# pminervini/hyperopt

Hardware: AMD Instinct MI355X
Metric: EI candidates scored/sec (x components) (higher is better)
Workload: dtype f64 (log-sum-exp: fp64 accumulation, fp32 exp2 of the shifted term, its argument from an fp32 block-local quadratic (mode 3); quantized: fp64 erf); 1 GPU; config 4: 100-D uniform space, 1e4-trial history, 1e7 candidates/suggest (lpdf roofline stress); parallelism=single

## Files before the change

### hyperopt_amd/_engine.py

```python
from __future__ import annotations

import ctypes as C
import os
import threading

import numpy as np

_HERE = os.path.dirname(os.path.abspath(__file__))
LIB_PATH = os.environ.get('TPE_ENGINE_LIB', os.path.join(_HERE, 'libtpe_engine.so'))

TPE_OK = 0
TPE_E_INVALID = -1
TPE_E_BOUNDS = -2
TPE_E_NEGATIVE = -3
TPE_E_NOMEM = -4
TPE_E_HIP = -5
TPE_E_NODEVICE = -6
TPE_E_INDEX = -7

GMM, LGMM, CAT = 0, 1, 2
HAS_LOW, HAS_HIGH, HAS_Q, PCHOICE = 1, 2, 4, 8
OBS_IDENT, OBS_LOG, OBS_LOG_CLIP_EXPLOW, OBS_LOG_CLIP_EPS = 0, 1, 2, 3
KIND_NAMES = ('lse_gmm', 'lse_lgmm', 'erf_gmm', 'erf_lgmm', 'categorical')

EXPORTS = (
    'tpe_version', 'tpe_device_count', 'tpe_create', 'tpe_destroy', 'tpe_last_error',
    'tpe_synchronize', 'tpe_split', 'tpe_parzen_fit', 'tpe_categorical_posterior',
    'tpe_lpdf', 'tpe_score', 'tpe_sample', 'tpe_plan_create', 'tpe_plan_destroy',
    'tpe_plan_num_levels', 'tpe_plan_set_history', 'tpe_plan_fit', 'tpe_plan_get_mixture',
    'tpe_plan_get_table',
    'tpe_plan_suggest', 'tpe_plan_suggest_shard', 'tpe_plan_merge', 'tpe_plan_score_candidates', 'tpe_plan_last_stats',
    'tpe_plan_profile', 'tpe_plan_profile_read', 'tpe_microbench', 'tpe_plan_get_results',
    'tpe_plan_results_device', 'tpe_plan_census', 'tpe_plan_fit_suggest',
    'tpe_plan_set_lattice', 'tpe_plan_update_history', 'tpe_plan_set_prune',
    'tpe_plan_sample_prior', 'tpe_plan_score_candidates_sorted', 'tpe_plan_census_n',
    'tpe_plan_tie_counts', 'tpe_plan_tab_wmax', 'tpe_plan_anneal', 'tpe_plan_anneal_trace',
    'tpe_plan_set_anneal_order', 'tpe_plan_tab_bound', 'tpe_plan_tab_hot',
    'tpe_plan_cand_dump', 'tpe_plan_draw_screen_stats', 'tpe_plan_score_points',
    'tpe_plan_sample_points', 'tpe_plan_topk_points', 'tpe_plan_gather_points',
    'tpe_plan_joint_fit', 'tpe_plan_joint_get_mixture', 'tpe_plan_joint_score_points',
    'tpe_plan_joint_sides', 'tpe_plan_joint_sample_points', 'tpe_math_probe',
    'tpe_plan_group_info', 'tpe_plan_group_fit', 'tpe_plan_group_get_mixture',
    'tpe_plan_group_score_points', 'tpe_plan_group_sides', 'tpe_plan_group_sample_points',
    'tpe_plan_group_batch_points',
    'tpe_plan_set_objectives', 'tpe_plan_pareto_get', 'tpe_plan_pareto_shape',
)

BATCH_MAX = 1024
MAX_OBJ = 8

SHARD_ALIGN = 8192


class EngineUnavailable(RuntimeError):
    """The HIP engine library or an MI355X (gfx950) device is not available."""


class EngineError(RuntimeError):
    pass


class TpeHp(C.Structure):
    _fields_ = [('family', C.c_int32), ('flags', C.c_uint32), ('obs_transform', C.c_int32),
                ('upper', C.c_int32), ('prior_mu', C.c_double), ('prior_sigma', C.c_double),
                ('low', C.c_double), ('high', C.c_double), ('q', C.c_double),
                ('cond_begin', C.c_int32), ('cond_count', C.c_int32),
                ('pprior_begin', C.c_int64)]


class TpeSpace(C.Structure):
    _fields_ = [('n_hp', C.c_int32), ('hp', C.POINTER(TpeHp)), ('n_cond', C.c_int32),
                ('cond_parent', C.POINTER(C.c_int32)), ('cond_branch', C.POINTER(C.c_int32)),
                ('n_pprior', C.c_int64), ('pprior', C.POINTER(C.c_double))]


RESULT_DTYPE = np.dtype([('score', '<f8'), ('value', '<f8'), ('index', '<i8'),
                         ('active', '<i4'), ('pad', '<i4')])
ANNEAL_TRACE_DTYPE = np.dtype([('row', '<i4'), ('rank', '<i4'), ('u', '<f8', (4,))])

_D = C.POINTER(C.c_double)
_lib = None
_lib_lock = threading.Lock()


def _share_hip_runtime():
    if os.environ.get('TPE_ENGINE_HIP_RUNTIME', '') == 'system':
        return
    import importlib.util
    try:
        spec = importlib.util.find_spec('torch')
    except (ImportError, ValueError):
        spec = None
    if spec is None or not spec.origin:
        return
    hip = os.path.join(os.path.dirname(spec.origin), 'lib', 'libamdhip64.so')
    if os.path.exists(hip):
        C.CDLL(hip, mode=C.RTLD_GLOBAL)


def load_library(path: str = LIB_PATH):
    global _lib
    with _lib_lock:
        if _lib is not None:
            return _lib
        if not os.path.exists(path):
            raise EngineUnavailable(
                'libtpe_engine.so not found at %s: build it with `make -C '
                'hyperopt_amd/csrc` or __graft_entry__.build()' % path)
        _share_hip_runtime()
        lib = C.CDLL(path)
        vp, i32, i64, u32, u64, dbl = C.c_void_p, C.c_int32, C.c_int64, C.c_uint32, C.c_uint64, C.c_double
        sig = {
            'tpe_version': (C.c_char_p, []),
            'tpe_device_count': (C.c_int, [C.POINTER(i32)]),
            'tpe_create': (C.c_int, [i32, C.POINTER(vp)]),
            'tpe_destroy': (C.c_int, [vp]),
            'tpe_last_error': (C.c_char_p, [vp]),
            'tpe_synchronize': (C.c_int, [vp]),
            'tpe_split': (C.c_int, [vp, _D, i64, dbl, i32, C.POINTER(C.c_uint8)]),
            'tpe_parzen_fit': (C.c_int, [vp, _D, i64, dbl, dbl, dbl, i32, _D, _D, _D]),
            'tpe_categorical_posterior': (C.c_int, [vp, C.POINTER(i64), i64, i32, dbl, _D, i32, _D]),
            'tpe_lpdf': (C.c_int, [vp, i32, _D, i64, _D, _D, _D, i64, dbl, dbl, dbl, u32, _D]),
            'tpe_score': (C.c_int, [vp, i32, _D, i64, _D, _D, _D, i64, _D, _D, _D, i64,
                                    dbl, dbl, dbl, u32, _D, _D, C.POINTER(i64), _D]),
            'tpe_sample': (C.c_int, [vp, i32, _D, _D, _D, i64, dbl, dbl, dbl, u32, u64, u64,
                                     i64, i64, _D]),
            'tpe_plan_create': (C.c_int, [vp, C.POINTER(TpeSpace), i64, C.POINTER(vp)]),
            'tpe_plan_destroy': (C.c_int, [vp]),
            'tpe_plan_num_levels': (C.c_int, [vp, C.POINTER(i32)]),
            'tpe_plan_set_history': (C.c_int, [vp, vp, vp, vp, i64, i32, vp]),
            'tpe_plan_update_history': (C.c_int, [vp, i64, i64, i64, vp, vp, i64, i64, vp, i32,
                                                  vp]),
            'tpe_plan_fit': (C.c_int, [vp, dbl, i32, dbl, i32, vp]),
            'tpe_plan_get_mixture': (C.c_int, [vp, i32, i32, _D, _D, _D, i64, C.POINTER(i64)]),
            'tpe_plan_get_table': (C.c_int, [vp, i32, i32, i32, vp, i64, C.POINTER(i64)]),
            'tpe_plan_suggest': (C.c_int, [vp, C.POINTER(u64), i64, i64, i64, i32, vp, i32, vp]),
            'tpe_plan_suggest_shard': (C.c_int, [vp, C.POINTER(u64), i64, i64, i64, i64, i32, vp,
                                                 i32, vp]),
            'tpe_plan_fit_suggest': (C.c_int, [vp, dbl, i32, dbl, i32, C.POINTER(u64), i64, i64,
                                               vp, i32, vp]),
            'tpe_plan_merge': (C.c_int, [vp, vp, i32, i32, vp, i32, vp]),
            'tpe_plan_score_candidates': (C.c_int, [vp, i32, _D, i64, _D, _D, C.POINTER(i64), _D]),
            'tpe_plan_score_candidates_sorted': (C.c_int, [vp, i32, i32, _D, i64, _D, _D,
                                                           C.POINTER(i64), _D]),
            'tpe_plan_score_points': (C.c_int, [vp, vp, i64, i64, vp, vp, vp, i32, vp]),
            'tpe_plan_sample_points': (C.c_int, [vp, u64, i64, i64, i64, vp, vp, vp, vp, i32, vp]),
            'tpe_plan_topk_points': (C.c_int, [vp, vp, vp, i64, i32, vp, i32, vp]),
            'tpe_plan_joint_fit': (C.c_int, [vp, vp]),
            'tpe_plan_joint_get_mixture': (C.c_int, [vp, i32, i32, _D, _D, _D, vp, i64,
                                                     C.POINTER(i64)]),
            'tpe_plan_joint_score_points': (C.c_int, [vp, vp, i64, i64, vp, vp, vp, vp, i32, vp]),
            'tpe_plan_joint_sides': (C.c_int, [vp, vp, vp, i64]),
            'tpe_plan_joint_sample_points': (C.c_int, [vp, u64, i64, i64, i64, vp, vp, vp, vp, vp,
                                                       vp, i32, vp]),
            'tpe_plan_group_info': (C.c_int, [vp, vp, C.POINTER(i32)]),
            'tpe_plan_group_fit': (C.c_int, [vp, vp]),
            'tpe_plan_group_get_mixture': (C.c_int, [vp, i32, i32, i32, _D, _D, _D, vp, i64,
                                                     C.POINTER(i64)]),
            'tpe_plan_group_score_points': (C.c_int, [vp, vp, i64, i64, vp, vp, vp, i32, vp]),
            'tpe_plan_group_sides': (C.c_int, [vp, i32, vp, vp, i64]),
            'tpe_plan_group_sample_points': (C.c_int, [vp, u64, i64, i64, i64, vp, vp, vp, vp, vp,
                                                       i32, vp]),
            'tpe_plan_group_batch_points': (C.c_int, [vp, vp, i64, i64, vp, i32, vp, vp, vp, i32,
                                                      vp]),
            'tpe_plan_gather_points': (C.c_int, [vp, vp, i64, vp, i32, vp, i32, vp]),
            'tpe_plan_set_objectives': (C.c_int, [vp, vp, i32, i64, i64, i64, i32, vp]),
            'tpe_plan_pareto_get': (C.c_int, [vp, vp, vp, vp, i64]),
            'tpe_plan_pareto_shape': (C.c_int, [vp, i64, i32, i64, C.POINTER(i64)]),
            'tpe_plan_last_stats': (C.c_int, [vp, _D, _D]),
            'tpe_plan_profile': (C.c_int, [vp, i32]),
            'tpe_plan_profile_read': (C.c_int, [vp, i32, _D, C.POINTER(i64), _D]),
            'tpe_microbench': (C.c_int, [vp, i32, _D]),
            'tpe_math_probe': (C.c_int, [vp, i32, _D, i64, _D]),
            'tpe_plan_get_results': (C.c_int, [vp, vp, i32, vp]),
            'tpe_plan_results_device': (vp, [vp]),
            'tpe_plan_census': (C.c_int, [vp, i32, C.POINTER(i64)]),
            'tpe_plan_census_n': (C.c_int, [vp, i32, C.POINTER(i64), i32]),
            'tpe_plan_tie_counts': (C.c_int, [vp, i32, vp]),
            'tpe_plan_tab_wmax': (C.c_int, [vp, i32, vp]),
            'tpe_plan_tab_bound': (C.c_int, [vp, i32, vp]),
            'tpe_plan_tab_hot': (C.c_int, [vp, i32, vp]),
            'tpe_plan_cand_dump': (C.c_int64, [vp, i32, i32, vp, vp]),
            'tpe_plan_draw_screen_stats': (C.c_int, [vp, vp]),
            'tpe_plan_set_lattice': (C.c_int, [vp, i32]),
            'tpe_plan_set_prune': (C.c_int, [vp, i32]),
            'tpe_plan_sample_prior': (C.c_int, [vp, C.POINTER(u64), i64, vp, i32, vp]),
            'tpe_plan_anneal': (C.c_int, [vp, dbl, dbl, C.POINTER(u64), i64, vp, i32, vp]),
            'tpe_plan_anneal_trace': (C.c_int, [vp, i32, vp]),
            'tpe_plan_set_anneal_order': (C.c_int, [vp, C.POINTER(i32), i32]),
        }
        for name, (res, args) in sig.items():
            fn = getattr(lib, name)
            fn.restype = res
            fn.argtypes = args
        _lib = lib
        return lib


def _seeds(seeds):
    seeds = [int(x) & (2 ** 64 - 1) for x in np.atleast_1d(np.asarray(seeds, dtype=object))]
    return np.fromiter(seeds, dtype=np.uint64, count=len(seeds))


def _dp(a):
    return None if a is None else a.ctypes.data_as(_D)


def _f64(a):
    return np.ascontiguousarray(a, dtype=np.float64)


class Engine(object):

    def __init__(self, device: int = 0):
        self.lib = load_library()
        n = C.c_int32(0)
        self.lib.tpe_device_count(C.byref(n))
        if n.value <= 0:
            raise EngineUnavailable('no HIP device visible (TPE engine needs an MI355X)')
        h = C.c_void_p()
        rc = self.lib.tpe_create(int(device), C.byref(h))
        if rc != TPE_OK:
            raise EngineUnavailable('tpe_create(%d) failed (%d): not a gfx950 device?' % (device, rc))
        self.h = h
        self.device = device
        self.lock = threading.RLock()

    def close(self):
        if getattr(self, 'h', None):
            self.lib.tpe_destroy(self.h)
            self.h = None

    def __del__(self):
        try:
            self.close()
        except Exception:
            pass

    def check(self, rc):
        if rc == TPE_OK:
            return
        msg = (self.lib.tpe_last_error(self.h) or b'').decode()
        if rc == TPE_E_BOUNDS:
            raise ValueError('low >= high', msg)
        if rc == TPE_E_NEGATIVE:
            raise ValueError('negative arg to lognormal_cdf', msg)
        if rc == TPE_E_INDEX:
            raise IndexError(msg)
        if rc == TPE_E_INVALID:
            raise ValueError(msg)
        raise EngineError('TPE engine error %d: %s' % (rc, msg))

    def synchronize(self):
        with self.lock:
            self.check(self.lib.tpe_synchronize(self.h))

    def microbench(self, which):
        r = C.c_double(0)
        with self.lock:
            self.check(self.lib.tpe_microbench(self.h, int(which), C.byref(r)))
        return r.value

    def math_probe(self, which, x):
        xa = _f64(x)
# ... 660 lines not shown
        idx = np.empty(max(int(k), 0), dtype=np.int32)
        with e.lock:
            e.check(e.lib.tpe_plan_topk_points(
                self.p, total.ctypes.data, None if el is None else el.ctypes.data, total.size,
                int(k), idx.ctypes.data, 0, stream))
        return idx

    def gather_points(self, vals, idx, k=None, ld=None, out=None, stream=None):
        e = self.engine
        if k is not None:
            with e.lock:
                e.check(e.lib.tpe_plan_gather_points(self.p, vals, int(ld), idx, int(k), out, 1,
                                                     stream))
            return None
        vals = _f64(vals)
        if vals.ndim != 2 or vals.shape[0] != self.n_hp:
            raise ValueError('configurations must be a [n_hp, M] array')
        idx = np.ascontiguousarray(idx, dtype=np.int32).ravel()
        res = np.empty((self.n_hp, idx.size))
        with e.lock:
            e.check(e.lib.tpe_plan_gather_points(self.p, vals.ctypes.data, vals.shape[1],
                                                 idx.ctypes.data, idx.size, res.ctypes.data, 0,
                                                 stream))
        return res

    def profile(self, capacity):
        e = self.engine
        with e.lock:
            e.check(e.lib.tpe_plan_profile(self.p, int(capacity)))

    def profile_read(self, kind):
        e = self.engine
        ms, n, pairs = C.c_double(0), C.c_int64(0), C.c_double(0)
        with e.lock:
            e.check(e.lib.tpe_plan_profile_read(self.p, int(kind), C.byref(ms), C.byref(n),
                                                C.byref(pairs)))
        return ms.value, n.value, pairs.value

    def set_lattice(self, enable):
        e = self.engine
        with e.lock:
            e.check(e.lib.tpe_plan_set_lattice(self.p, int(bool(enable))))

    def set_prune(self, mode):
        mode = 3 if mode is True else int(mode)
        e = self.engine
        with e.lock:
            e.check(e.lib.tpe_plan_set_prune(self.p, mode))

    def census(self, enable, n=7):
        if not 0 <= n <= 13:
            raise ValueError('the census has 13 counters')
        e = self.engine
        out = (C.c_int64 * 13)()
        with e.lock:
            e.check(e.lib.tpe_plan_census_n(self.p, int(bool(enable)), out, int(n)))
        return tuple(int(v) for v in out[:n])

    def tie_counts(self, n_suggest):
        e = self.engine
        out = np.empty((int(n_suggest), self.n_hp), dtype=np.int32)
        with e.lock:
            e.check(e.lib.tpe_plan_tie_counts(self.p, int(n_suggest), out.ctypes.data))
        return out

    def tab_wmax(self, n_suggest):
        e = self.engine
        with e.lock:
            w = e.lib.tpe_plan_tab_wmax(self.p, int(n_suggest), None)
            e.check(min(w, 0))
            out = np.empty((int(n_suggest), self.n_hp, w), dtype=np.float64)
            e.check(e.lib.tpe_plan_tab_wmax(self.p, int(n_suggest), out.ctypes.data))
        return out

    def tab_bound(self, hp):
        e = self.engine
        with e.lock:
            n = e.lib.tpe_plan_tab_bound(self.p, int(hp), None)
            e.check(min(n, 0))
            out = np.empty(n, dtype=np.float64)
            e.check(e.lib.tpe_plan_tab_bound(self.p, int(hp), out.ctypes.data))
        return out

    def tab_hot(self, n_suggest):
        e = self.engine
        out = np.empty((int(n_suggest), self.n_hp, 18), dtype=np.float64)
        with e.lock:
            e.check(e.lib.tpe_plan_tab_hot(self.p, int(n_suggest), out.ctypes.data))
        return out

    def cand_dump(self, s, hp):
        e = self.engine
        with e.lock:
            n = e.lib.tpe_plan_cand_dump(self.p, int(s), int(hp), None, None)
            e.check(int(min(n, 0)))
            vals = np.empty(n, dtype=np.float64)
            pos = np.empty(n, dtype=np.int32)
            e.check(int(min(e.lib.tpe_plan_cand_dump(self.p, int(s), int(hp), vals.ctypes.data,
                                                     pos.ctypes.data), 0)))
        return vals, pos

    def draw_screen_stats(self):
        e = self.engine
        out = np.zeros(3, dtype=np.int64)
        with e.lock:
            e.check(e.lib.tpe_plan_draw_screen_stats(self.p, out.ctypes.data))
        return int(out[0]), int(out[1]), int(out[2])

    def last_stats(self):
        e = self.engine
        ms, pairs = C.c_double(0), C.c_double(0)
        with e.lock:
            e.check(e.lib.tpe_plan_last_stats(self.p, C.byref(ms), C.byref(pairs)))
        return ms.value, pairs.value


_default = {}
_default_lock = threading.Lock()


def default_engine(device: int | None = None) -> Engine:
    if device is None:
        device = int(os.environ.get('LOCAL_RANK', '0'))
    with _default_lock:
        eng = _default.get(device)
        if eng is None:
            eng = Engine(device)
            _default[device] = eng
        return eng
```

### hyperopt_amd/csrc/tpe_engine.hip

```cpp
#include <hip/hip_runtime.h>

#include <algorithm>
#include <cmath>
#include <cstdlib>
#include <cstdio>
#include <cstring>
#include <string>
#include <vector>

#include "tpe_anneal.hpp"
#include "tpe_group_plan.hpp"
#include "tpe_internal.hpp"
#include "tpe_level_plan.hpp"
#include "tpe_pareto_plan.hpp"
#include "tpe_switches.hpp"

using namespace tpe;
static_assert(sizeof(AnnealTrace) == sizeof(tpe_anneal_trace), "layout");

struct tpe_engine {
  int32_t device = 0;
  hipStream_t stream = nullptr;
  static constexpr int kAux = 4;
  hipStream_t aux[kAux] = {};
  std::string err;
  tpe_plan *op = nullptr;
};

struct tpe_plan : PlanShape {
  tpe_engine *eng = nullptr;
  int32_t P = 0;
  int64_t ncap = 0;
  int32_t last_nb = -1;
  std::vector<double> pprior;
  std::vector<int32_t> level_off;
  tpe_hp *d_hps = nullptr;
  int32_t *d_cp = nullptr, *d_cb = nullptr, *d_level_hps = nullptr, *d_all_hps = nullptr;
  int32_t *d_level_off = nullptr;
  double *d_pprior = nullptr;
  double *d_losses = nullptr, *d_vals = nullptr;
  uint8_t *d_active = nullptr, *d_below = nullptr;
  double *d_mw = nullptr, *d_mmu = nullptr, *d_msig = nullptr, *d_scratch = nullptr;
  unsigned char *d_sortbuf = nullptr;
  int64_t scap = 0;
  MixInfo *d_info = nullptr;
  Coef *d_coef = nullptr;
  Coef32 *d_coef32 = nullptr;
  CoefM *d_coefm = nullptr;
  CoefM8 *d_coefm8 = nullptr;
  float4 *d_coefe = nullptr;
  CoefM8 *d_coefmh = nullptr;
  TabHdr *d_tab_hdr = nullptr;
  TabPanel *d_tab = nullptr;
  double *d_tab_max = nullptr;
  double *d_tab_wmax = nullptr;
  int32_t *d_tie_list = nullptr;
  int32_t *d_tie_cnt = nullptr;
  int32_t tab_pstride = 0;
  double *d_tab_bound = nullptr;
  TabHot *d_tab_hot = nullptr;
  DrawZone *d_draw_zone = nullptr;
  unsigned long long *d_screen_stats = nullptr;
  bool tab_built = false;
  bool graph_tab = false;
  int64_t n = 0;
  int64_t s_cap = 0;
  Partial *d_results = nullptr;
  tpe_result *h_results = nullptr;
  size_t h_results_cap = 0;
  uint64_t *h_flag = nullptr;
  uint64_t seq = 0;
  bool pub_fired = false;
  uint64_t *d_seeds = nullptr;
  Partial *d_partial = nullptr;
  size_t partial_cap = 0;
  unsigned long long *d_census = nullptr;
  bool census = false;
  uint32_t *d_ticket = nullptr;
  std::vector<uint64_t> h_seeds;
  bool has_erf = false;
  LatInfo *d_lat_info = nullptr;
  double2 *d_lat = nullptr;
  bool lattice_on = true;
  int32_t prune_mode = 3;
  hipEvent_t ev_fork = nullptr, ev_join[8] = {};
  double *d_ext = nullptr, *d_lb = nullptr, *d_la = nullptr;
  size_t ext_cap = 0;
  double *d_pt_vals = nullptr, *d_pt_terms = nullptr, *d_pt_total = nullptr;
  uint8_t *d_pt_act = nullptr;
  int32_t *d_pt_idx = nullptr;
  uint32_t *d_pt_count = nullptr;
  size_t pt_cap = 0;
  void *d_pt_tab = nullptr;
  void *d_tk = nullptr;
  int32_t *d_tk_idx = nullptr;
  double *d_cand = nullptr;
  int32_t *d_cpos = nullptr;
  size_t cand_cap = 0;
  std::vector<JointDim> jdims;
  std::vector<int32_t> jdim_of_hp;
  int32_t j_slots = 0;
  int64_t j_nopt = 0;
  bool joint_ok = false;
  int32_t jK[2] = {0, 0};
  double fit_pw = 1.0;
  int32_t fit_lf = 0;
  JointDim *d_jdims = nullptr;
  int32_t *d_jdim_of_hp = nullptr, *d_jrows = nullptr, *d_jcount = nullptr, *d_jcomp = nullptr;
  JointSide *d_jside = nullptr;
  uint64_t *d_jkeys = nullptr;
  double *d_jw = nullptr, *d_jcw = nullptr, *d_jcmu = nullptr, *d_jcsig = nullptr;
  double *d_jtab = nullptr, *d_joptlog = nullptr, *d_jpick = nullptr, *d_joptcdf = nullptr;
  size_t joptcdf_cap = 0;
  void *d_jdraw = nullptr;
  double *d_jsides = nullptr, *d_jjoint = nullptr;
  size_t jpt_cap = 0;
  int64_t jpt_m = 0;
  GroupPartition gpart;
  GroupLayout glay;
  bool group_ready = false, group_ok = false;
  int32_t gkb_max = 0;
  JointDim *d_gdims = nullptr;
  GroupDesc *d_ggroups = nullptr;
  int32_t *d_gdim_of_hp = nullptr, *d_ggroup_of_hp = nullptr, *d_grows = nullptr;
  int32_t *d_gcount = nullptr, *d_gcomp = nullptr;
  JointSide *d_gside = nullptr;
  uint64_t *d_gkeys = nullptr;
  double *d_gw = nullptr, *d_gcw = nullptr, *d_gcmu = nullptr, *d_gcsig = nullptr;
  double *d_gtab = nullptr, *d_goptlog = nullptr, *d_gpick = nullptr, *d_goptcdf = nullptr;
  size_t goptcdf_cap = 0;
  void *d_gdraw = nullptr;
  double *d_gsides = nullptr, *d_gjoint = nullptr;
  size_t gpt_cap = 0;
  int64_t gpt_m = 0;
  double *d_bt_ja = nullptr, *d_bt_score = nullptr, *d_bt_gain = nullptr, *d_bt_trace = nullptr;
  uint8_t *d_bt_gact = nullptr, *d_bt_state = nullptr;
  void *d_bt_slot = nullptr, *d_bt_rec = nullptr;
  int32_t *d_bt_idx = nullptr;
  size_t bt_cap = 0, bt_trace_cap = 0;
  int64_t bt_m = -1;
  hipEvent_t ev0 = nullptr, ev1 = nullptr;
  struct Prof {
// ... 20 lines not shown
    }
  };
  StepKey graph_key, pending_key;
  bool graph_ok = false, pending = false;
  int32_t mom_w = 0;
  bool mom_h = false;
  bool graph_mom_h = false;
  int32_t graph_mom_w = 0;
  HistPatch pend{};
  bool has_pend = false;
  uint64_t *d_an_keys = nullptr;
  int32_t *d_an_idx = nullptr;
  int32_t *d_an_T = nullptr;
  int32_t *d_an_hporder = nullptr;
  AnnealTrace *d_an_trace = nullptr;
  int64_t an_cap = 0, an_nsug = 0;
  bool an_ready = false;
  bool an_order = false;
  double *d_obj = nullptr;
  int32_t *d_pcount = nullptr;
  int32_t obj_M = 0;
  int64_t obj_n = 0;
  int64_t pareto_n = -1;
  int64_t pareto_force = 0;
  hipGraph_t graph = nullptr;
  hipGraphExec_t graph_exec = nullptr;
  std::vector<hipGraphNode_t> fit_nodes, draw_nodes;
  std::vector<hipKernelNodeParams> fit_params, draw_params;
  std::vector<FitArgs> fit_args0;
  std::vector<ScoreArgs> draw_args0;
};

namespace {

#define CKH(expr)                                                        \
  do {                                                                   \
    hipError_t e_ = (expr);                                              \
    if (e_ != hipSuccess) {                                              \
      return fail(h, TPE_E_HIP, std::string(#expr) + ": " + hipGetErrorString(e_)); \
    }                                                                    \
  } while (0)

int fail(tpe_engine *h, int code, const std::string &msg) {
  if (h) h->err = msg;
  return code;
}

template <typename T>
hipError_t dalloc(T **p, size_t count) {
  *p = nullptr;
  if (count == 0) count = 1;
  return hipMalloc((void **)p, count * sizeof(T));
}

void dfree(void *p) {
  if (p) (void)hipFree(p);
}

void graph_reset(tpe_plan *p) {
  if (p->graph_exec) (void)hipGraphExecDestroy(p->graph_exec);
  if (p->graph) (void)hipGraphDestroy(p->graph);
  p->graph_exec = nullptr;
  p->graph = nullptr;
  p->graph_ok = p->pending = false;
  p->fit_nodes.clear(); p->draw_nodes.clear();
  p->fit_params.clear(); p->draw_params.clear();
  p->fit_args0.clear(); p->draw_args0.clear();
}

hipStream_t pick_stream(tpe_engine *h, void *s) {
  return s ? (hipStream_t)s : h->stream;
}

void plan_free_buffers(tpe_plan *p) {
  void *bufs[] = {p->d_an_keys, p->d_an_idx, p->d_an_T, p->d_an_hporder, p->d_an_trace,
                  p->d_hps, p->d_cp, p->d_cb, p->d_level_hps, p->d_all_hps, p->d_pprior,
                  p->d_level_off,
                  p->d_losses, p->d_vals, p->d_active, p->d_below, p->d_mw, p->d_mmu,
                  p->d_msig, p->d_scratch, p->d_info, p->d_coef, p->d_results, p->d_seeds,
                  p->d_partial, p->d_ext, p->d_lb, p->d_la, p->d_cand, p->d_cpos,
                  p->d_ticket, p->d_sortbuf, p->d_census, p->d_lat_info, p->d_lat, p->d_coef32, p->d_coefm,
                  p->d_coefm8, p->d_coefe, p->d_coefmh, p->d_tab_hdr, p->d_tab,
                  p->d_tab_max, p->d_tab_wmax, p->d_tie_list, p->d_tie_cnt, p->d_tab_bound,
                  p->d_tab_hot, p->d_draw_zone, p->d_screen_stats, p->d_pt_vals, p->d_pt_terms,
                  p->d_pt_total, p->d_pt_act, p->d_pt_idx, p->d_pt_count, p->d_pt_tab, p->d_tk,
                  p->d_tk_idx, p->d_jdims, p->d_jdim_of_hp, p->d_jrows, p->d_jcount, p->d_jcomp,
                  p->d_jside, p->d_jkeys, p->d_jw, p->d_jcw, p->d_jcmu, p->d_jcsig, p->d_jtab,
                  p->d_joptlog, p->d_jpick, p->d_joptcdf, p->d_jdraw, p->d_jsides, p->d_jjoint,
                  p->d_gdims, p->d_ggroups, p->d_gdim_of_hp, p->d_ggroup_of_hp, p->d_grows,
                  p->d_gcount, p->d_gcomp, p->d_gside, p->d_gkeys, p->d_gw, p->d_gcw, p->d_gcmu,
                  p->d_gcsig, p->d_gtab, p->d_goptlog, p->d_gpick, p->d_goptcdf, p->d_gdraw,
                  p->d_gsides, p->d_gjoint, p->d_bt_ja, p->d_bt_score, p->d_bt_gain,
                  p->d_bt_trace, p->d_bt_gact, p->d_bt_state, p->d_bt_slot, p->d_bt_rec,
                  p->d_bt_idx, p->d_obj, p->d_pcount};
  for (void *b : bufs) dfree(b);
  if (p->h_results) (void)hipHostFree(p->h_results);
  p->h_results = nullptr;
  p->h_results_cap = 0;
  if (p->h_flag) (void)hipHostFree(p->h_flag);
  p->h_flag = nullptr;
  if (p->ev0) (void)hipEventDestroy(p->ev0);
  if (p->ev1) (void)hipEventDestroy(p->ev1);
  if (p->ev_fork) (void)hipEventDestroy(p->ev_fork);
  for (auto e : p->ev_join) if (e) (void)hipEventDestroy(e);
  for (auto &pr : p->prof) {
    for (auto e : pr.a) (void)hipEventDestroy(e);
    for (auto e : pr.b) (void)hipEventDestroy(e);
    pr.a.clear(); pr.b.clear(); pr.pairs.clear(); pr.n = 0;
  }
}

int validate_space(tpe_engine *h, const tpe_space *sp) {
  if (!sp || sp->n_hp <= 0 || !sp->hp) return fail(h, TPE_E_INVALID, "empty space");
  for (int i = 0; i < sp->n_hp; ++i) {
    const tpe_hp &x = sp->hp[i];
    if (x.family < TPE_GMM || x.family > TPE_CAT)
      return fail(h, TPE_E_INVALID, "hp " + std::to_string(i) + ": bad family");
    if (x.family == TPE_CAT && x.upper <= 0)
      return fail(h, TPE_E_INVALID, "hp " + std::to_string(i) + ": categorical upper <= 0");
    if (x.family != TPE_CAT) {
      const bool hl = x.flags & TPE_HAS_LOW, hh = x.flags & TPE_HAS_HIGH;
      if (hl != hh)
        return fail(h, TPE_E_INVALID, "hp " + std::to_string(i) + ": one-sided truncation");
      if (hl && !(x.low < x.high))
        return fail(h, TPE_E_BOUNDS, "low >= high");
      if (!(x.prior_sigma > 0))
        return fail(h, TPE_E_INVALID, "hp " + std::to_string(i) + ": prior_sigma <= 0");
    }
    if (x.cond_count < 0 || x.cond_begin < 0 || x.cond_begin + x.cond_count > sp->n_cond)
      return fail(h, TPE_E_INVALID, "hp " + std::to_string(i) + ": bad condition range");
    for (int c = 0; c < x.cond_count; ++c) {
      const int par = sp->cond_parent[x.cond_begin + c];
      if (par < 0 || par >= sp->n_hp || par == i)
        return fail(h, TPE_E_INVALID, "hp " + std::to_string(i) + ": bad condition parent");
    }
    if ((x.flags & TPE_PCHOICE) &&
        (x.pprior_begin < 0 || x.pprior_begin + x.upper > sp->n_pprior))
      return fail(h, TPE_E_INVALID, "hp " + std::to_string(i) + ": bad pchoice prior");
  }
  return TPE_OK;
}

LatInfo lattice_of(const tpe_hp &x) {
  LatInfo L{0, 0, 0, 0};
  const int k = score_kind(x);
  if (k != KIND_ERF_G && k != KIND_ERF_L) return L;
  if (!(x.flags & TPE_HAS_LOW) || !(x.flags & TPE_HAS_HIGH) || !(x.q > 0.0)) return L;
  double lo = x.low, hi = x.high;
  if (k == KIND_ERF_L) {
    lo = std::exp(lo);
    hi = std::exp(hi);
  }
  const double a = std::rint(lo / x.q) - 2.0, b = std::rint(hi / x.q) + 2.0;
  if (!(std::fabs(a) < 1e15 && std::fabs(b) < 1e15) || b - a + 1.0 > (double)kLatMaxR)
    return L;
  L.j0 = (int64_t)a;
  L.R = (int32_t)(b - a + 1.0);
  return L;
}

int compute_levels(tpe_engine *h, tpe_plan *p) {
  std::vector<int> lev(p->P, -1);
  for (int iter = 0; iter <= p->P; ++iter) {
    bool changed = false;
    for (int i = 0; i < p->P; ++i) {
      const tpe_hp &x = p->hps[i];
// ... 12 lines not shown
  for (int i = 0; i < p->P; ++i) {
    if (lev[i] < 0 || lev[i] > p->P) return fail(h, TPE_E_INVALID, "cyclic conditions");
    nl = std::max(nl, lev[i] + 1);
  }
  p->levels.assign(nl, {});
  for (int lat : {1, 0})
    for (int kind : {KIND_ERF_L, KIND_ERF_G})
      for (int i = 0; i < p->P; ++i)
        if (score_kind(p->hps[i]) == kind && (lattice_of(p->hps[i]).R > 0) == (lat == 1))
          p->levels[lev[i]].push_back(i);
  for (int kind : {KIND_LSE_L, KIND_LSE_G, KIND_CAT})
    for (int i = 0; i < p->P; ++i)
      if (score_kind(p->hps[i]) == kind) p->levels[lev[i]].push_back(i);
  p->level_off.assign(nl + 1, 0);
  for (int l = 0; l < nl; ++l)
    p->level_off[l + 1] = p->level_off[l] + (int)p->levels[l].size();
  return TPE_OK;
}

int plan_build(tpe_engine *h, const tpe_space *sp, int64_t max_trials, tpe_plan *p) {
  int rc = validate_space(h, sp);
  if (rc) return rc;
  if (max_trials < 0) return fail(h, TPE_E_INVALID, "max_trials < 0");
  p->eng = h;
  p->P = sp->n_hp;

  p->hps.assign(sp->hp, sp->hp + sp->n_hp);
  p->cond_parent.assign(sp->cond_parent, sp->cond_parent + sp->n_cond);
  p->cond_branch.assign(sp->cond_branch, sp->cond_branch + sp->n_cond);
  p->pprior.assign(sp->pprior, sp->pprior + sp->n_pprior);
  rc = compute_levels(h, p);
  if (rc) return rc;
  p->ncap = std::max<int64_t>(max_trials, 1);
  int64_t kcap = p->ncap + 1;
  for (const auto &x : p->hps)
    if (x.family == TPE_CAT) kcap = std::max<int64_t>(kcap, x.upper);
  kcap = (kcap + kCoefBlock - 1) / kCoefBlock * kCoefBlock;
  p->kcap = kcap;
  for (const auto &x : p->hps) {
    const int k = score_kind(x);
    if (k == KIND_ERF_G || k == KIND_ERF_L) p->has_erf = true;
  }
  const int64_t slots = 2 * (int64_t)p->P;
  p->lat.assign(p->P, LatInfo{0, 0, 0, 0});
  int64_t lat_total = 0;
  for (int i = 0; i < p->P; ++i) {
    p->lat[i] = lattice_of(p->hps[i]);
    p->lat[i].off = lat_total;
    lat_total += p->lat[i].R;
  }
  CKH(hipSetDevice(h->device));
  CKH(dalloc(&p->d_lat_info, p->P));
  CKH(dalloc(&p->d_lat, std::max<int64_t>(1, lat_total)));
  CKH(dalloc(&p->d_hps, p->P));
  CKH(dalloc(&p->d_cp, p->cond_parent.size()));
  CKH(dalloc(&p->d_cb, p->cond_branch.size()));
  CKH(dalloc(&p->d_pprior, p->pprior.size()));
  CKH(dalloc(&p->d_level_hps, p->P));
  CKH(dalloc(&p->d_all_hps, p->P));
  CKH(dalloc(&p->d_level_off, p->level_off.size()));
  CKH(dalloc(&p->d_losses, p->ncap));
  CKH(dalloc(&p->d_vals, (size_t)p->ncap * p->P));
  CKH(dalloc(&p->d_active, (size_t)p->ncap * p->P));
  CKH(dalloc(&p->d_below, p->ncap));
  CKH(dalloc(&p->d_mw, (size_t)slots * kcap));
  CKH(dalloc(&p->d_mmu, (size_t)slots * kcap));
  CKH(dalloc(&p->d_msig, (size_t)slots * kcap));
  CKH(dalloc(&p->d_scratch, (size_t)slots * kcap));
  p->scap = p->ncap + 1;
  CKH(dalloc(&p->d_sortbuf, (size_t)slots * 16 * p->scap));
  CKH(dalloc(&p->d_info, slots));
  CKH(dalloc(&p->d_census, kCensus));
  CKH(hipMemset(p->d_census, 0, kCensus * sizeof(unsigned long long)));
  CKH(dalloc(&p->d_coef, (size_t)slots * kcap));
  CKH(dalloc(&p->d_coef32, (size_t)slots * (kcap / kCoefBlock)));
  CKH(dalloc(&p->d_coefm, (size_t)slots * mom_stride(kcap)));
  CKH(dalloc(&p->d_coefm8, (size_t)slots * (kcap / kCoefBlock)));
  CKH(dalloc(&p->d_coefe, (size_t)slots * (kcap / kCoefBlock)));
  CKH(dalloc(&p->d_coefmh, (size_t)slots * mom_stride(kcap)));
  CKH(dalloc(&p->d_tab_hdr, (size_t)slots));
  CKH(hipMemset(p->d_tab_hdr, 0, (size_t)slots * sizeof(TabHdr)));
  CKH(dalloc(&p->d_tab, (size_t)slots * kTabMaxPanels));
  CKH(dalloc(&p->d_tab_bound, (size_t)p->P * kBndCells));
  p->act_frac.assign(p->P, 1.0);
  for (const auto &lv : p->levels)
    for (int i : lv) {
      const tpe_hp &x = p->hps[i];
      if (x.cond_count == 0) continue;
      double f = 0.0;
      for (int c = 0; c < x.cond_count; ++c) {
        const int par = p->cond_parent[x.cond_begin + c];
        const tpe_hp &y = p->hps[par];
        f += p->act_frac[par] / (y.family == TPE_CAT ? std::max(1, (int)y.upper) : 1);
      }
      p->act_frac[i] = std::min(1.0, f);
    }
  p->finish();
  CKH(hipEventCreate(&p->ev0));
  CKH(hipEventCreate(&p->ev1));
  CKH(hipEventCreateWithFlags(&p->ev_fork, hipEventDisableTiming));
  for (auto &e : p->ev_join) CKH(hipEventCreateWithFlags(&e, hipEventDisableTiming));
  std::vector<int32_t> lh;
  for (auto &l : p->levels) lh.insert(lh.end(), l.begin(), l.end());
  std::vector<int32_t> all(p->P);
  for (int i = 0; i < p->P; ++i) all[i] = i;
  hipStream_t st = h->stream;
  CKH(hipMemcpyAsync(p->d_hps, p->hps.data(), p->P * sizeof(tpe_hp), hipMemcpyHostToDevice, st));
  CKH(hipMemcpyAsync(p->d_lat_info, p->lat.data(), p->P * sizeof(LatInfo), hipMemcpyHostToDevice,
                     st));
  if (!p->cond_parent.empty()) {
    CKH(hipMemcpyAsync(p->d_cp, p->cond_parent.data(), p->cond_parent.size() * 4, hipMemcpyHostToDevice, st));
    CKH(hipMemcpyAsync(p->d_cb, p->cond_branch.data(), p->cond_branch.size() * 4, hipMemcpyHostToDevice, st));
  }
  if (!p->pprior.empty())
    CKH(hipMemcpyAsync(p->d_pprior, p->pprior.data(), p->pprior.size() * 8, hipMemcpyHostToDevice, st));
  CKH(hipMemcpyAsync(p->d_level_hps, lh.data(), lh.size() * 4, hipMemcpyHostToDevice, st));
  CKH(hipMemcpyAsync(p->d_all_hps, all.data(), all.size() * 4, hipMemcpyHostToDevice, st));
  CKH(hipMemcpyAsync(p->d_level_off, p->level_off.data(), p->level_off.size() * 4,
                     hipMemcpyHostToDevice, st));
  CKH(hipMemsetAsync(p->d_info, 0, slots * sizeof(MixInfo), st));
  CKH(hipStreamSynchronize(st));
  return TPE_OK;
}

int ensure_suggest_state(tpe_engine *h, tpe_plan *p, int64_t n_sug, size_t partials) {
  if (n_sug > p->s_cap || partials > p->partial_cap) graph_reset(p);
  if (n_sug > p->s_cap) {
    dfree(p->d_results);
    dfree(p->d_seeds);
    dfree(p->d_ticket);
    p->d_results = nullptr;
    p->d_seeds = nullptr;
    p->d_ticket = nullptr;
    CKH(dalloc(&p->d_results, (size_t)n_sug * p->P));
    CKH(dalloc(&p->d_seeds, n_sug));
    CKH(dalloc(&p->d_ticket, (size_t)n_sug * p->P + 1));
    CKH(hipMemset(p->d_ticket, 0, ((size_t)n_sug * p->P + 1) * sizeof(uint32_t)));
    dfree(p->d_tab_max);
    p->d_tab_max = nullptr;
    CKH(dalloc(&p->d_tab_max, (size_t)n_sug * p->P));
    dfree(p->d_tie_cnt);
    p->d_tie_cnt = nullptr;
    CKH(dalloc(&p->d_tie_cnt, (size_t)n_sug * p->P));
    CKH(hipMemset(p->d_tie_cnt, 0xff, (size_t)n_sug * p->P * sizeof(int32_t)));
    dfree(p->d_tab_hot);
    p->d_tab_hot = nullptr;
    CKH(dalloc(&p->d_tab_hot, (size_t)n_sug * p->P));
    dfree(p->d_draw_zone);
    p->d_draw_zone = nullptr;
    CKH(dalloc(&p->d_draw_zone, (size_t)n_sug * p->P));
    if (!p->d_screen_stats) {
      CKH(dalloc(&p->d_screen_stats, 2));
      CKH(hipMemset(p->d_screen_stats, 0, 2 * sizeof(unsigned long long)));
    }
    p->s_cap = n_sug;
  }
  if (partials > p->partial_cap) {
    dfree(p->d_partial);
    p->d_partial = nullptr;
    CKH(dalloc(&p->d_partial, partials));
    dfree(p->d_tab_wmax);
    p->d_tab_wmax = nullptr;
    CKH(dalloc(&p->d_tab_wmax, partials * 8));
    CKH(hipMemset(p->d_tab_wmax, 0xff, partials * 8 * sizeof(double)));
    dfree(p->d_tie_list);
    p->d_tie_list = nullptr;
// ... 86 lines not shown
  a.results = p->d_results;
  a.partial = p->d_partial;
  a.ticket = p->d_ticket;
  a.census = p->census ? p->d_census : nullptr;
  a.kcap = p->kcap;
  a.n_hp = p->P;
  a.n_suggest = (int32_t)n_sug;
  a.lat_info = p->d_lat_info;
  a.lat = p->d_lat;
  a.lse_mom = p->mom_w;
  a.lse_momh = p->mom_w == 16 && p->mom_h ? 1 : 0;
  a.l2_warm = 0;
  a.lse_tight = 1;
  a.tab_hdr = p->d_tab_hdr;
  a.tab = p->d_tab;
  a.tab_max = p->d_tab_max;
  a.tab_wmax = p->d_tab_wmax;
  a.tie_list = p->d_tie_list;
  a.tie_cnt = p->d_tie_cnt;
  a.tab_tie = switches().table_tie();
  a.tab_bound = p->d_tab_bound;
  a.tab_hot = p->d_tab_hot;
  return a;
}

FitVariant plan_fit_variant(const tpe_plan *p, bool moments) {
  return fit_variant(*p, switches(), p->n, fit_small(p->n), moments);
}

FitArgs fit_args(tpe_plan *p, int32_t n_below, double prior_weight, int32_t lf,
                 const FitVariant &f) {
  p->mom_w = f.mom_w;
  p->mom_h = f.mom_h;
  p->tab_built = false;
  p->joint_ok = false;
  p->group_ok = false;
  p->fit_pw = prior_weight;
  p->fit_lf = lf;
  FitArgs a{};
  a.hps = p->d_hps;
  a.vals = p->d_vals;
  a.active = p->d_active;
  a.losses = p->d_losses;
  a.n = p->n;
  a.ld = p->ncap;
  a.n_below = n_below;
  a.lf = lf;
  a.prior_weight = prior_weight;
  a.pprior = p->d_pprior;
  a.mw = p->d_mw;
  a.mmu = p->d_mmu;
  a.msig = p->d_msig;
  a.info = p->d_info;
  a.coef = p->d_coef;
  a.coef32 = p->d_coef32;
  a.coefm = p->mom_w == 16 ? p->d_coefm : nullptr;
  a.coefm8 = p->mom_w == 8 ? p->d_coefm8 : nullptr;
  a.coefmh = p->mom_h ? p->d_coefmh : nullptr;
  a.coefe = p->d_coefe;
  a.kcap = p->kcap;
  a.ob = p->d_scratch;
  a.tmp = p->d_scratch;
  a.sortbuf = p->d_sortbuf;
  a.scap = p->scap;
  return a;
}

int flush_patch(tpe_engine *h, tpe_plan *p, hipStream_t st) {
  if (!p->has_pend) return TPE_OK;
  p->has_pend = false;
  CKH(launch_hist_patch(p->pend, p->d_vals, p->d_active, p->d_losses, st));
  return TPE_OK;
}
int fit_launch(tpe_engine *h, tpe_plan *p, const FitArgs &a, int32_t n_hp, hipStream_t st) {
  CKH(launch_fit(a, n_hp, st, p->has_pend ? &p->pend : nullptr));
  p->has_pend = false;
  return TPE_OK;
}

int table_build(tpe_engine *h, tpe_plan *p, hipStream_t st) {
  if (p->tab_built) return TPE_OK;
  CKH(launch_table_build(p->d_hps, p->P, p->d_info, p->d_coef, p->kcap, p->d_tab_hdr, p->d_tab,
                         p->census ? p->d_census : nullptr, st,
                         switches().table_prefilter ? p->d_tab_bound : nullptr));
  p->tab_built = true;
  return TPE_OK;
}

int score_launch(tpe_engine *h, tpe_plan *p, ScoreArgs a, bool has_erf, int64_t cn,
                 hipStream_t sg, bool record, int classes = 7) {
  tpe_plan::Prof *pr = nullptr;
  if (record && p->prof_cap > 0) {
    pr = &p->prof[0];
    if (pr->n >= p->prof_cap) pr = nullptr;
  }
  if (pr) CKH(hipEventRecord(pr->a[pr->n], sg));
  if (a.tab_on == 1 && (classes & 1)) {
    const int rc = table_build(h, p, sg);
    if (rc) return rc;
    p->tab_pstride = a.pstride;
  }
  CKH(launch_score(a, has_erf, sg, switches().side_streams ? h->aux[1] : nullptr, p->ev_join[1],
                   p->ev_join[2], classes));
  if (pr) {
    CKH(hipEventRecord(pr->b[pr->n], sg));
    pr->pairs[pr->n] = (double)cn * (double)a.n_suggest;
    pr->n++;
  }
  return TPE_OK;
}

StepShape step_shape(const tpe_plan *p, int64_t n_sug, int64_t n_cand, int64_t cand_begin,
                     int64_t n_total, int32_t last_nb, const FitVariant &f) {
  StepShape s;
  s.n_sug = n_sug;
  s.n_cand = n_cand;
  s.cand_begin = cand_begin;
  s.n_total = n_total;
  s.below = below_class(last_nb >= 0 ? (int64_t)last_nb + 1 : p->kcap);
  s.fit = f;
  s.prune_mode = p->prune_mode;
  s.lattice_on = p->lattice_on;
  s.screen_run = step_screen_run(switches());
  return s;
}

int run_level(tpe_engine *h, tpe_plan *p, int level, const StepShape &s, hipStream_t st) {
  const LevelPlan lp = plan_level(*p, switches(), s, level);
  const int64_t n_sug = s.n_sug;
  const int32_t n_level = lp.n_level, n_lat = lp.n_lat;
  const int32_t *lvl = p->d_level_hps + p->level_off[level];
  if (lp.empty) {
    if (n_level > 0) CKH(launch_merge(lvl, n_level, (int32_t)n_sug, p->P, 0, nullptr, p->d_results, st));
    return TPE_OK;
  }
  ScoreArgs la = base_args(p, n_sug);
  la.level_hps = lvl;
  la.n_slots = n_level;
  la.slot_rows = lp.slot_rows;
  la.compact = lp.compact ? 1 : 0;
  auto lat_bracket = [&](hipStream_t sl, auto launch) -> int {
    tpe_plan::Prof *pr = nullptr;
    if (p->prof_cap > 0 && p->prof[1].n < p->prof_cap) pr = &p->prof[1];
    if (pr) CKH(hipEventRecord(pr->a[pr->n], sl));
    CKH(launch());
    if (pr) {
      CKH(hipEventRecord(pr->b[pr->n], sl));
      pr->pairs[pr->n] = (double)level;
      pr->n++;
    }
    return TPE_OK;
  };
  auto lattice = [&](hipStream_t sl) -> int {
    return lat_bracket(sl, [&] {
      return launch_lattice(la, p->levels[level].data(), p->hps.data(), p->lat.data(), n_lat,
                            p->d_lat, sl, lp.lat_rows);
    });
  };
  const bool lat_side = lp.lat == LatRun::Side;
  bool lat_pending = lp.lat == LatRun::Deferred;
  if (lp.lat == LatRun::InOrder || lat_side) {
    hipStream_t sl = st;
    if (lat_side) {
      sl = h->aux[0];
      CKH(hipEventRecord(p->ev_fork, st));
      CKH(hipStreamWaitEvent(sl, p->ev_fork, 0));
    }
    const int lrc = lattice(sl);
    if (lat_side) {
      const hipError_t e1 = hipEventRecord(p->ev_join[0], sl);
      if (lrc) {
        if (e1 == hipSuccess) (void)hipStreamWaitEvent(st, p->ev_join[0], 0);
        return lrc;
      }
      if (e1 != hipSuccess) return fail(h, TPE_E_HIP, "lattice side stream join event");
    } else if (lrc) {
      return lrc;
    }
  }
  bool joined = !lat_side;
  auto chunks = [&]() -> int {
  for (const ChunkPlan &c : lp.chunks) {
    const int64_t cn = c.cn;
    if (c.grid.pstride < 0) return fail(h, TPE_E_INVALID, "level slots not grouped by lpdf kind");
    int rc = ensure_suggest_state(h, p, n_sug, (size_t)n_sug * p->P * c.grid.pstride);
    if (rc) return rc;
    rc = ensure_cand(h, p, (size_t)std::max<int64_t>(1, n_sug * n_level * cn));
    if (rc) return rc;
    ScoreArgs a = base_args(p, n_sug);
    copy_groups(a, c.grid);
    a.compact = lp.compact ? 1 : 0;
    a.cand = p->d_cand;
    a.cand_sstride = (int64_t)n_level * cn;
    a.n_cand = cn;
    a.cand_begin = s.cand_begin + c.c0;
    a.accumulate = c.accumulate ? 1 : 0;
    a.level_hps = lvl;
    a.n_slots = n_level;
    a.slot_rows = lp.slot_rows;
    a.cand_slot0 = 0;
    for (int i = 0; i < kInlineSeeds && i < n_sug; ++i) a.seed_inline[i] = p->h_seeds[i];
    a.n_inline_seeds = (int32_t)std::min<int64_t>(n_sug, kInlineSeeds);
    a.lse_pos = c.lse_pos;
    a.sort_log2 = c.sort_log2;
    a.lookup_draw = c.lookup_draw;
    a.lse_prune = c.lse_prune;
// ... 2215 lines not shown
  CKH(hipDeviceSynchronize());
  if (counts) {
    unsigned long long c[kCensus];
    CKH(hipMemcpy(c, p->d_census, sizeof(c), hipMemcpyDeviceToHost));
    for (int i = 0; i < kCensus && i < n_counts; ++i) counts[i] = (int64_t)c[i];
  }
  CKH(hipMemset(p->d_census, 0, kCensus * sizeof(unsigned long long)));
  p->census = enable != 0;
  return TPE_OK;
}

int tpe_plan_tie_counts(tpe_plan_t p, int32_t n_suggest, int32_t *counts) {
  if (!p || !counts || n_suggest < 0) return TPE_E_INVALID;
  tpe_engine *h = p->eng;
  if (n_suggest > p->s_cap) return fail(h, TPE_E_INVALID, "more suggestions than the last call's");
  CKH(hipSetDevice(h->device));
  CKH(hipDeviceSynchronize());
  if (n_suggest > 0)
    CKH(hipMemcpy(counts, p->d_tie_cnt, (size_t)n_suggest * p->P * sizeof(int32_t),
                  hipMemcpyDeviceToHost));
  return TPE_OK;
}

int tpe_plan_tab_wmax(tpe_plan_t p, int32_t n_suggest, double *out) {
  if (!p || n_suggest < 0) return TPE_E_INVALID;
  tpe_engine *h = p->eng;
  const size_t row = (size_t)p->tab_pstride * 8;
  if (!out) return (int)row;
  if (n_suggest > p->s_cap || (size_t)n_suggest * p->P * p->tab_pstride > p->partial_cap)
    return fail(h, TPE_E_INVALID, "more suggestions than the last call's");
  CKH(hipSetDevice(h->device));
  CKH(hipDeviceSynchronize());
  if (n_suggest > 0 && row > 0)
    CKH(hipMemcpy(out, p->d_tab_wmax, (size_t)n_suggest * p->P * row * sizeof(double),
                  hipMemcpyDeviceToHost));
  return TPE_OK;
}

int64_t tpe_plan_cand_dump(tpe_plan_t p, int32_t s, int32_t hp, double *values, int32_t *positions) {
  if (!p) return TPE_E_INVALID;
  tpe_engine *h = p->eng;
  if (p->dump_level < 0 || p->dump_cn <= 0) return fail(h, TPE_E_INVALID, "no sorted draw yet");
  if (!values && !positions) return p->dump_cn;
  const std::vector<int32_t> &lv = p->levels[p->dump_level];
  int64_t slot = -1;
  for (size_t i = 0; i < lv.size(); ++i)
    if (lv[i] == hp) slot = (int64_t)i;
  if (slot < 0 || s < 0 || s >= p->dump_nsug)
    return fail(h, TPE_E_INVALID, "hp / suggestion not of the last sorted draw");
  CKH(hipSetDevice(h->device));
  CKH(hipDeviceSynchronize());
  const int64_t off = (int64_t)s * p->dump_sstride + slot * p->dump_cn;
  if (values)
    CKH(hipMemcpy(values, p->d_cand + off, (size_t)p->dump_cn * sizeof(double), hipMemcpyDeviceToHost));
  if (positions)
    CKH(hipMemcpy(positions, p->d_cpos + off, (size_t)p->dump_cn * sizeof(int32_t),
                  hipMemcpyDeviceToHost));
  return p->dump_cn;
}

int tpe_plan_tab_bound(tpe_plan_t p, int32_t hp, double *out) {
  if (!p) return TPE_E_INVALID;
  if (!out) return kBndCells;
  tpe_engine *h = p->eng;
  if (hp < 0 || hp >= p->P) return fail(h, TPE_E_INVALID, "bad args");
  if (!table_hp(p->hps[hp])) return fail(h, TPE_E_INVALID, "hp has no Chebyshev table");
  if (!switches().table_prefilter) return fail(h, TPE_E_INVALID, "no bound lattice: the prefilter is off");
  CKH(hipSetDevice(h->device));
  CKH(hipDeviceSynchronize());
  const int rc = table_build(h, p, h->stream);
  if (rc) return rc;
  TabHdr th[2];
  CKH(hipMemcpyAsync(th, p->d_tab_hdr + 2 * (int64_t)hp, sizeof(th), hipMemcpyDeviceToHost,
                     h->stream));
  CKH(hipStreamSynchronize(h->stream));
  for (const TabHdr &t : th)
    if (!(t.P > 0 && t.ncert == (uint32_t)t.P))
      return fail(h, TPE_E_INVALID, "Chebyshev table not certified");
  CKH(hipMemcpy(out, p->d_tab_bound + (int64_t)hp * kBndCells, kBndCells * sizeof(double),
                hipMemcpyDeviceToHost));
  return TPE_OK;
}

int tpe_plan_draw_screen_stats(tpe_plan_t p, int64_t *out) {
  if (!p || !out) return TPE_E_INVALID;
  tpe_engine *h = p->eng;
  out[0] = out[1] = out[2] = 0;
  if (!p->d_screen_stats) return TPE_OK;
  CKH(hipSetDevice(h->device));
  CKH(hipDeviceSynchronize());
  unsigned long long v[2];
  CKH(hipMemcpy(v, p->d_screen_stats, sizeof(v), hipMemcpyDeviceToHost));
  CKH(hipMemset(p->d_screen_stats, 0, sizeof(v)));
  out[0] = (int64_t)(v[0] >> 40);
  out[1] = (int64_t)v[1];
  out[2] = (int64_t)(v[0] & ((1ull << 40) - 1));
  return TPE_OK;
}

int tpe_plan_tab_hot(tpe_plan_t p, int32_t n_suggest, double *out) {
  static_assert(sizeof(TabHot) == (2 + 2 * kHotIv) * sizeof(double), "y_lo, y_hi, lo[], hi[]");
  if (!p || !out || n_suggest < 0) return TPE_E_INVALID;
  tpe_engine *h = p->eng;
  if (n_suggest > p->s_cap) return fail(h, TPE_E_INVALID, "more suggestions than the last call's");
  CKH(hipSetDevice(h->device));
  CKH(hipDeviceSynchronize());
  if (n_suggest > 0)
    CKH(hipMemcpy(out, p->d_tab_hot, (size_t)n_suggest * p->P * sizeof(TabHot),
                  hipMemcpyDeviceToHost));
  return TPE_OK;
}

int tpe_plan_sample_prior(tpe_plan_t p, const uint64_t *seeds, int64_t n_sug, tpe_result *out,
                          int32_t out_on_device, void *stream) {
  if (!p) return TPE_E_INVALID;
  tpe_engine *h = p->eng;
  if (n_sug <= 0 || !seeds) return fail(h, TPE_E_INVALID, "bad args");
  CKH(hipSetDevice(h->device));
  hipStream_t st = pick_stream(h, stream);
  int rc = ensure_suggest_state(h, p, n_sug, 1);
  if (rc) return rc;
  CKH(hipMemcpyAsync(p->d_seeds, seeds, n_sug * 8, hipMemcpyHostToDevice, st));
  PriorArgs a{};
  a.hps = p->d_hps;
  a.n_hp = p->P;
  a.n_levels = (int32_t)p->levels.size();
  a.level_hps = p->d_level_hps;
  a.level_off = p->d_level_off;
  a.cond_parent = p->d_cp;
  a.cond_branch = p->d_cb;
  a.pprior = p->d_pprior;
  a.seeds = p->d_seeds;
  a.results = p->d_results;
  CKH(launch_prior(a, (int32_t)n_sug, st));
  p->last_nsug = n_sug;
  if (!out_on_device) {
    rc = copy_results(h, p, n_sug, out, 0, st);
    if (rc) return rc;
    return TPE_OK;
  }
  return copy_results(h, p, n_sug, out, out_on_device, st);
}

int tpe_plan_set_anneal_order(tpe_plan_t p, const int32_t *hp_order, int32_t n_hp) {
  if (!p) return TPE_E_INVALID;
  tpe_engine *h = p->eng;
  if (!hp_order || n_hp != p->P) return fail(h, TPE_E_INVALID, "anneal order: one entry per hp");
  std::vector<int32_t> pos(p->P, -1);
  for (int k = 0; k < n_hp; ++k) {
    const int hp = hp_order[k];
    if (hp < 0 || hp >= p->P || pos[hp] >= 0)
      return fail(h, TPE_E_INVALID, "anneal order: not a permutation of the hps");
    pos[hp] = k;
  }
  for (int hp = 0; hp < p->P; ++hp) {
    const tpe_hp &x = p->hps[hp];
    for (int c = 0; c < x.cond_count; ++c)
      if (pos[p->cond_parent[x.cond_begin + c]] > pos[hp])
        return fail(h, TPE_E_INVALID, "anneal order: an hp before the choice that leads to it");
  }
  CKH(hipSetDevice(h->device));
  p->an_order = false;
  if (!p->d_an_hporder) CKH(dalloc(&p->d_an_hporder, p->P));
  CKH(hipDeviceSynchronize());
  CKH(hipMemcpy(p->d_an_hporder, hp_order, (size_t)n_hp * 4, hipMemcpyHostToDevice));
  p->an_order = true;
// ... 179 lines not shown
```

### hyperopt_amd/csrc/tpe_internal.hpp

```cpp
#pragma once
#include <hip/hip_runtime.h>
#include <stdint.h>

#include "../../include/tpe_engine.h"

namespace tpe {

constexpr double kEPS = 1e-12;
constexpr int kFitThreads = 1024;
constexpr int kScoreThreads = 256;
constexpr int kMaxLeaves = 160;

enum { KIND_LSE_G = 0, KIND_LSE_L = 1, KIND_ERF_G = 2, KIND_ERF_L = 3, KIND_CAT = 4,
       KIND_LAT = 5, KIND_LSE_G1 = 6, KIND_LSE_L1 = 7, KIND_LSE_GW = 8, KIND_LSE_LW = 9,
       KIND_LSE_GW1 = 10, KIND_LSE_LW1 = 11 };
constexpr int64_t kWaveRowSplitMax = (int64_t)1 << 18;

__host__ __device__ constexpr bool kind_lse(int k) {
  return k == KIND_LSE_G || k == KIND_LSE_L || k == KIND_LSE_G1 || k == KIND_LSE_L1 ||
         k == KIND_LSE_GW || k == KIND_LSE_LW || k == KIND_LSE_GW1 || k == KIND_LSE_LW1;
}
__host__ __device__ constexpr bool kind_logn(int k) {
  return k == KIND_LSE_L || k == KIND_LSE_L1 || k == KIND_LSE_LW || k == KIND_LSE_LW1 ||
         k == KIND_ERF_L;
// ... 268 lines not shown
hipError_t launch_score(const ScoreArgs &a, bool has_erf, hipStream_t st,
                        hipStream_t side = nullptr, hipEvent_t ev_fork = nullptr,
                        hipEvent_t ev_join = nullptr, int classes = 7);
int score_classes(const ScoreArgs &a);
constexpr int kLatThreads = 256;
struct LatJob {
  tpe_hp H;
  LatInfo L;
  int32_t hp;
  int32_t pad;
};
constexpr int kLatJobs = 8;
struct LatJobs {
  LatJob job[kLatJobs];
  int32_t n_jobs;
  int32_t draw_gx;
  int32_t draw_blocks;
  int32_t compact;
  int32_t n_lat;
  int32_t pad[3];
};
constexpr int kFuseTab = 32;
hipError_t launch_lattice(const ScoreArgs &a, const int32_t *hps_of_level, const tpe_hp *hps,
                          const LatInfo *lat, int32_t n_lat, double2 *lat_out, hipStream_t st,
                          int32_t lat_rows);
hipError_t launch_lattice_draw(const ScoreArgs &a, const int32_t *hps_of_level, const tpe_hp *hps,
                               const LatInfo *lat, int32_t n_lat, double2 *lat_out,
                               hipStream_t st, int32_t lat_rows);
constexpr int kTabCap = 2048;
hipError_t launch_draw(const ScoreArgs &a, bool table, hipStream_t st);
constexpr int kSortedBlock = TPE_SHARD_ALIGN;
constexpr int kSortLog2Large = 13, kSortLog2Small = 12;
static_assert((1 << kSortLog2Large) == kSortedBlock, "largest sort block");
__host__ __device__ constexpr int sort_log2_for(int64_t n_total) {
  return n_total > kWaveRowSplitMax ? kSortLog2Large : kSortLog2Small;
}
hipError_t launch_draw_sorted(const ScoreArgs &a, bool small_table, bool fast, int32_t *pos_out,
                              hipStream_t st, int64_t max_blocks = INT64_MAX);
hipError_t launch_draw_pruned(const ScoreArgs &a, bool small_table, bool fast, int32_t *pos_out,
                              hipStream_t st);
constexpr int kZoneMax = 6;
constexpr int kZoneEdges = 2 * kZoneMax - 2;
constexpr double kScreenMargin = 1.6e-5;
constexpr int kGuideBitsMax = 10;
struct __attribute__((aligned(16))) DrawZone {
  int32_t nz;
  int32_t gbits;
  double gap_lo[kZoneMax - 1];
  double gap_hi[kZoneMax - 1];
  double thr[kFuseTab][kZoneEdges];
  uint64_t thrI[kFuseTab][kZoneEdges];
  uint64_t pickB[kFuseTab];
  uint16_t guide[1 << kGuideBitsMax];
  double tcdf[kFuseTab], tbase[kFuseTab], tmass[kFuseTab];
  unsigned char tmode[kFuseTab];
};
hipError_t launch_draw_zone(const ScoreArgs &a, DrawZone *zones, int32_t tiles, double margin,
                            int32_t guide_bits, hipStream_t st);
constexpr int kScreenRunMax = 16;
hipError_t launch_draw_screened(const ScoreArgs &a, int32_t *pos_out, const DrawZone *zones,
                                unsigned long long *stats, bool integer, int32_t run,
                                hipStream_t st);
bool is_screen_draw_kernel_fn(const void *f);
bool is_screen_run_kernel_fn(const void *f);
hipError_t launch_table_pilot(const ScoreArgs &a, hipStream_t st);
static_assert(kSortedBlock == TPE_SHARD_ALIGN, "shard alignment is the sorted-draw block");
hipError_t launch_sort_ext(const ScoreArgs &a, const double *src, int32_t *pos_out,
                           hipStream_t st);
hipError_t launch_bucket(const ScoreArgs &a, int32_t slot_begin, int32_t *pos_out, hipStream_t st);
hipError_t launch_publish(const void *src, void *dst, size_t bytes, uint64_t *flag, uint64_t seq,
                          hipStream_t st);
hipError_t launch_merge(const int32_t *level_hps, int32_t n_slots,
                        int32_t n_suggest, int32_t n_hp, int32_t world,
                        const Partial *gathered, Partial *results,
                        hipStream_t st, Partial *out2 = nullptr);
hipError_t launch_sample(const tpe_hp *hp_dev, const double *mw,
                         const double *mmu, const double *msig,
                         const MixInfo *info, uint64_t seed, uint64_t stream,
                         int64_t offset, int64_t n, double *out,
                         hipStream_t st);

hipError_t launch_micro(int which, int blocks, int iters, double *sink, hipStream_t st);
hipError_t launch_math_probe(int which, const double *x, int64_t n, double *out, hipStream_t st);
hipError_t launch_table_build(const tpe_hp *hps, int32_t n_hp, const MixInfo *info,
                              const Coef *coef, int64_t kcap, TabHdr *hdr, TabPanel *tab,
                              unsigned long long *census, hipStream_t st, double *bound = nullptr);

constexpr int kPatchVals = 192;
constexpr int kPatchLoss = 16;
struct HistPatch {
  int64_t row0, n_rows, loss0, n_loss, ld;
  int32_t P;
  int32_t pad;
  double vals[kPatchVals];
  double losses[kPatchLoss];
  uint8_t active[kPatchVals];
};
hipError_t launch_hist_patch(const HistPatch &h, double *vals, uint8_t *active, double *losses,
                             hipStream_t st);

struct PriorArgs {
  const tpe_hp *hps;
  int32_t n_hp;
  int32_t n_levels;
  const int32_t *level_hps;
  const int32_t *level_off;
  const int32_t *cond_parent;
  const int32_t *cond_branch;
  const double *pprior;
  const uint64_t *seeds;
  Partial *results;
};
hipError_t launch_prior(const PriorArgs &a, int32_t n_suggest, hipStream_t st);

struct PointsArgs {
  const tpe_hp *hps;
  const int32_t *level_hps;
  const int32_t *cond_parent;
  const int32_t *cond_branch;
  const MixInfo *info;
  const Coef *coef;
  int64_t kcap;
  const double *vals;
  int64_t m, ld;
  uint8_t *active;
  double *terms;
  double *total;
  int64_t act_ld, term_ld;
  int32_t *idx;
  uint32_t *count;
  int32_t n_hp;
  int32_t pad;
};
hipError_t launch_points(const PointsArgs &a, hipStream_t st);
hipError_t launch_points_score(const PointsArgs &a, hipStream_t st);

template <int CAP> struct DrawTableT;
struct SampleArgs {
  PointsArgs P;
  double *out;
  const double *mw, *mmu, *msig;
  DrawTableT<kTabCap> *tab;
  uint64_t seed;
  int64_t begin;
};
size_t sample_tables_bytes(int32_t n_hp);
hipError_t launch_sample_points(const SampleArgs &s, hipStream_t st);

struct JointDim {
  int32_t hp;
  int32_t kind;
  int32_t slot;
  int32_t upper;
  int64_t opt_off;
};
__host__ __device__ constexpr int joint_slots(int kind) {
  return kind == KIND_CAT ? 4 : (kind == KIND_ERF_G || kind == KIND_ERF_L) ? 2 : 1;
}
constexpr int kJointFields = 3;
__host__ __device__ constexpr int64_t joint_stride(int32_t n_dim) {
  return (int64_t)kCoefBlock * (1 + kJointFields * (int64_t)n_dim);
}
struct JointSide {
  double tot;
  double a1;
};
struct JointFitArgs {
  const tpe_hp *hps;
  const JointDim *dims;
// ... 213 lines not shown
```

### hyperopt_amd/csrc/tpe_kernels.hip

```cpp
#include <math.h>

#include <algorithm>
#include <cstdlib>

#include "tpe_draw.hpp"

namespace tpe {

constexpr int kSortMax = 8192;

constexpr int kDrawThreads = 256;
constexpr int kWideDrawThreads = 1024;
template <bool TAB>
__global__ __launch_bounds__(kDrawThreads) void k_draw(ScoreArgs A) {
  if constexpr (TAB) {
    __shared__ DrawTable T;
    draw_block<kTabCap>(A, blockIdx.x, blockIdx.y, blockIdx.z, T, (int64_t)gridDim.x * blockDim.x);
  } else {
    const int s = blockIdx.z;
    const int slot = row_slot(A, s, 0, A.n_slots, blockIdx.y);
    if (slot < 0) return;
    const int hp = A.level_hps[slot];
    const tpe_hp H = A.hps[hp];
    if (!A.compact && !hp_active(H, A.results + (int64_t)s * A.n_hp, A.cond_parent, A.cond_branch))
      return;
    const int64_t sb = 2 * (int64_t)hp;
    const double *bw = A.mw + sb * A.kcap, *bmu = A.mmu + sb * A.kcap, *bsg = A.msig + sb * A.kcap;
    const uint64_t seed = suggestion_seed(A, s);
    double *out = const_cast<double *>(A.cand) + (int64_t)s * A.cand_sstride + (int64_t)slot * A.n_cand;
    const int64_t stride = (int64_t)gridDim.x * blockDim.x;
#pragma unroll 1
    for (int64_t li = (int64_t)blockIdx.x * blockDim.x + threadIdx.x; li < A.n_cand; li += stride)
      out[li] = draw_one_ool(A.hps + hp, A.info + sb, bw, bmu, bsg, seed,
                             (uint64_t)(A.cand_begin + li), (uint32_t)hp);
  }
}

template <int CAP, int NT, bool EXT, bool FAST = false>
__device__ __forceinline__ void sorted_block(const ScoreArgs &A, int32_t *__restrict__ pos_out,
                                             const double *__restrict__ src,
                                             SortedDrawLds<CAP, NT> &L) {
  const int s = blockIdx.z;
  const int slot = row_slot(A, s, 0, A.n_slots, blockIdx.y);
  if (slot < 0) return;
  const int hp = A.level_hps[slot];
  if (!A.force_active && !A.compact &&
      !hp_active(A.hps[hp], A.results + (int64_t)s * A.n_hp, A.cond_parent, A.cond_branch))
    return;
  const int kind = slot_kind(A, slot);
  if (!EXT && (kind == KIND_CAT || kind == KIND_LAT) && lookup_inline(A, A.info[2 * hp].K)) return;
  sorted_block_body<CAP, NT, EXT, FAST>(
      A, slot, s, (int64_t)blockIdx.x << A.sort_log2,
      kind_lse(kind) || kind == KIND_ERF_G || kind == KIND_ERF_L, kind_logn(kind), pos_out, src,
      L);
}

constexpr int kSortThreads = 512;
template <int CAP>
__global__ __launch_bounds__(kSortThreads) __attribute__((amdgpu_waves_per_eu(CAP <= kFuseTab ? 2 : 1)))
void k_draw_sorted(ScoreArgs A, int32_t *__restrict__ pos_out) {
  __shared__ SortedDrawLds<CAP, kSortThreads> L;
  sorted_block<CAP, kSortThreads, false>(A, pos_out, nullptr, L);
}
template <int CAP>
__global__ __launch_bounds__(kSortThreads) __attribute__((amdgpu_waves_per_eu(CAP <= kFuseTab ? 4 : 1)))
void k_draw_sorted_fast(ScoreArgs A, int32_t *__restrict__ pos_out) {
  __shared__ SortedDrawLds<CAP, kSortThreads> L;
  sorted_block<CAP, kSortThreads, false, true>(A, pos_out, nullptr, L);
}

template <int CAP>
__global__ __launch_bounds__(kWideDrawThreads) void k_draw_sorted_wide(ScoreArgs A,
                                                                       int32_t *__restrict__ pos_out) {
  __shared__ SortedDrawLds<CAP, kWideDrawThreads> L;
  sorted_block<CAP, kWideDrawThreads, false>(A, pos_out, nullptr, L);
}
template <int CAP>
__global__ __launch_bounds__(kWideDrawThreads) void k_draw_sorted_wide_fast(
    ScoreArgs A, int32_t *__restrict__ pos_out) {
  __shared__ SortedDrawLds<CAP, kWideDrawThreads> L;
  sorted_block<CAP, kWideDrawThreads, false, true>(A, pos_out, nullptr, L);
}

__global__ __launch_bounds__(kDrawThreads) void k_sort_ext(ScoreArgs A, const double *__restrict__ src,
                                                           int32_t *__restrict__ pos_out) {
  __shared__ SortedDrawLds<1, kDrawThreads> L;
  sorted_block<1, kDrawThreads, true>(A, pos_out, src, L);
}
// ... 545 lines not shown
  if (a.n_slots <= 0 || a.n_suggest <= 0 || a.n_cand <= 0) return hipSuccess;
  const int64_t sbk = (int64_t)1 << a.sort_log2;
  const unsigned gx = (unsigned)std::min<int64_t>((a.n_cand + sbk - 1) / sbk, max_blocks);
  const dim3 g(gx, (unsigned)a.slot_rows, a.n_suggest);
  const bool wide = (int64_t)gx * a.slot_rows * a.n_suggest <= 2 * kNumCUs;
  if (wide) {
    if (fast) {
      if (small_table) k_draw_sorted_wide_fast<kFuseTab><<<g, kWideDrawThreads, 0, st>>>(a, pos_out);
      else k_draw_sorted_wide_fast<kTabCap><<<g, kWideDrawThreads, 0, st>>>(a, pos_out);
    } else {
      if (small_table) k_draw_sorted_wide<kFuseTab><<<g, kWideDrawThreads, 0, st>>>(a, pos_out);
      else k_draw_sorted_wide<kTabCap><<<g, kWideDrawThreads, 0, st>>>(a, pos_out);
    }
  } else if (fast) {
    if (small_table) k_draw_sorted_fast<kFuseTab><<<g, kSortThreads, 0, st>>>(a, pos_out);
    else k_draw_sorted_fast<kTabCap><<<g, kSortThreads, 0, st>>>(a, pos_out);
  } else if (small_table) {
    k_draw_sorted<kFuseTab><<<g, kSortThreads, 0, st>>>(a, pos_out);
  } else {
    k_draw_sorted<kTabCap><<<g, kSortThreads, 0, st>>>(a, pos_out);
  }
  return hipGetLastError();
}

hipError_t launch_sort_ext(const ScoreArgs &a, const double *src, int32_t *pos_out,
                           hipStream_t st) {
  if (a.n_slots <= 0 || a.n_suggest != 1 || a.n_cand <= 0) return hipSuccess;
  const int64_t sbk = (int64_t)1 << a.sort_log2;
  const unsigned gx = (unsigned)((a.n_cand + sbk - 1) / sbk);
  k_sort_ext<<<dim3(gx, a.n_slots, 1), kDrawThreads, 0, st>>>(a, src, pos_out);
  return hipGetLastError();
}

hipError_t launch_bucket(const ScoreArgs &a, int32_t slot_begin, int32_t *pos_out, hipStream_t st) {
  if (a.n_slots <= slot_begin || a.n_suggest <= 0 || a.n_cand <= 0) return hipSuccess;
  const unsigned gx = (unsigned)((a.n_cand + kSortMax - 1) / kSortMax);
  const unsigned rows = (unsigned)std::min(a.n_slots - slot_begin, a.slot_rows);
  k_bucket<<<dim3(gx, rows, a.n_suggest), 1024, (size_t)kSortMax * 9, st>>>(
      a, slot_begin, pos_out);
  return hipGetLastError();
}

__global__ __launch_bounds__(256) void k_publish(const uint64_t *__restrict__ src,
                                                 uint64_t *__restrict__ dst, int64_t n_words,
                                                 uint64_t *__restrict__ flag, uint64_t seq) {
  for (int64_t i = threadIdx.x; i < n_words; i += blockDim.x) dst[i] = src[i];
  __syncthreads();
  if (threadIdx.x == 0) {
    __builtin_amdgcn_fence(__ATOMIC_RELEASE, "");
    __hip_atomic_store(flag, seq, __ATOMIC_RELAXED, __HIP_MEMORY_SCOPE_SYSTEM);
  }
}

hipError_t launch_publish(const void *src, void *dst, size_t bytes, uint64_t *flag, uint64_t seq,
                          hipStream_t st) {
  k_publish<<<1, 256, 0, st>>>(static_cast<const uint64_t *>(src), static_cast<uint64_t *>(dst),
                               (int64_t)(bytes / 8), flag, seq);
  return hipGetLastError();
}

hipError_t launch_merge(const int32_t *level_hps, int32_t n_slots, int32_t n_suggest,
                        int32_t n_hp, int32_t world, const Partial *gathered,
                        Partial *results, hipStream_t st, Partial *out2) {
  if (n_slots <= 0 || n_suggest <= 0) return hipSuccess;
  k_merge<<<dim3(n_slots, n_suggest), 64, 0, st>>>(level_hps, n_slots, n_suggest, n_hp, world,
                                                   gathered, results, out2);
  return hipGetLastError();
}

hipError_t launch_sample(const tpe_hp *hp_dev, const double *mw, const double *mmu,
                         const double *msig, const MixInfo *info, uint64_t seed,
                         uint64_t stream, int64_t offset, int64_t n, double *out,
                         hipStream_t st) {
  if (n <= 0) return hipSuccess;
  const int64_t blocks = (n + 255) / 256;
  k_sample<<<(unsigned)blocks, 256, 0, st>>>(hp_dev, mw, mmu, msig, info, seed, (uint32_t)stream,
                                             offset, n, out);
  return hipGetLastError();
}

constexpr int kTabThreads = 256;
constexpr double kTabSkip = 64.0;

struct TabAcc {
  double m, s;
};
__device__ __forceinline__ void tab_add(TabAcc &a, double t) {
  const double mn = fmax(a.m, ceil(t));
  a.s = ldexp(a.s, (int)fmax(a.m - mn, -2100.0));
  a.m = mn;
  a.s += exp2(t - (mn == -INFINITY ? 0.0 : mn));
}
__device__ __forceinline__ void tab_merge(TabAcc &a, const TabAcc &b) {
  const double M = fmax(a.m, b.m);
  const double ms = M == -INFINITY ? 0.0 : M;
  a.s = ldexp(a.s, (int)fmax(a.m - ms, -2100.0)) + ldexp(b.s, (int)fmax(b.m - ms, -2100.0));
  a.m = M;
}
__device__ __forceinline__ TabAcc tab_wave_sum(TabAcc a) {
#pragma unroll
  for (int o = 32; o > 0; o >>= 1) {
    const TabAcc b{__shfl_xor(a.m, o, 64), __shfl_xor(a.s, o, 64)};
    tab_merge(a, b);
  }
  return a;
}

__global__ __launch_bounds__(kTabThreads) void k_table_build(
    const tpe_hp *__restrict__ hps, const MixInfo *__restrict__ info,
    const Coef *__restrict__ coef, int64_t kcap, TabHdr *__restrict__ hdr,
    TabPanel *__restrict__ tab, unsigned long long *__restrict__ census) {
  const int slot = blockIdx.y, p = blockIdx.x, tid = threadIdx.x;
  const tpe_hp H = hps[slot >> 1];
  if (!table_hp(H)) return;
  const MixInfo mi = info[slot];
  const int K = mi.K;
  if (K < 1 || K > kcap) return;
  const double *__restrict__ cf = reinterpret_cast<const double *>(coef + (int64_t)slot * kcap);
  __shared__ double red[4];
  __shared__ TabAcc acc[16][16];
  __shared__ TabAcc cert[2][4];
  __shared__ double fn[kTabNodes], cn[kTabNodes];
  __shared__ unsigned live_n;
  double a2 = 0.0;
  for (int k = tid; k < K; k += kTabThreads) a2 = fmax(a2, -cf[coef_off(k, 2)]);
#pragma unroll
  for (int o = 32; o > 0; o >>= 1) a2 = fmax(a2, __shfl_xor(a2, o, 64));
  if ((tid & 63) == 0) red[tid >> 6] = a2;
  if (tid == 0) live_n = 0u;
  __syncthreads();
  a2 = fmax(fmax(red[0], red[1]), fmax(red[2], red[3]));
  const double L2E = 1.4426950408889634;
  const double y_lo = H.low - H.prior_mu, y_hi = H.high - H.prior_mu;
  const double sig = sqrt(0.5 * L2E / a2);
  const double Pd = ceil((y_hi - y_lo) / (2.0 * sig));
  if (!(Pd >= 1.0 && Pd <= (double)kTabMaxPanels)) return;
  const int P = (int)Pd;
  if (p >= P) return;
  const double w = (y_hi - y_lo) / Pd, Hh = 0.5 * w;
  if (p == 0 && tid == 0) {
    hdr[slot].y_lo = y_lo;
    hdr[slot].inv_w = 1.0 / w;
    hdr[slot].P = P;
  }
  const double pl = y_lo + w * (double)p, ph = y_lo + w * (double)(p + 1), pc = pl + Hh;
  double thr = -INFINITY;
  if (mi.probe >= 0 && mi.probe < K) {
    const double x = cf[coef_off(mi.probe, 0)], y = cf[coef_off(mi.probe, 1)],
                 z = cf[coef_off(mi.probe, 2)];
    const double t0 = fma(z, pl * pl, fma(y, pl, x)), t1 = fma(z, ph * ph, fma(y, ph, x));
    const double tm = fmin(t0, t1);
    if (tm == tm) thr = tm - kTabSkip;
  }
  const int j = tid & 15, l = tid >> 4;
  const double yn = pc + Hh * cospi((double)(2 * j + 1) / 32.0), yn2 = yn * yn;
  TabAcc a{-INFINITY, 0.0};
  unsigned nlive = 0;
  const int nb = (K + kCoefBlock - 1) / kCoefBlock;
  for (int b = l; b < nb; b += 16) {
    const float4 e = reinterpret_cast<const float4 *>(cf)[(int64_t)b * 16 + 12];
    const double d = fmax(0.0, fmax((double)e.x - ph, pl - (double)e.y));
    const double bound = (double)e.z - (double)fabsf(e.w) * d * d;
    if (bound < thr) continue;
    const double *__restrict__ blk = cf + (int64_t)b * (4 * kCoefBlock);
    double t[kCoefBlock], mx = -INFINITY;
#pragma unroll
    for (int i = 0; i < kCoefBlock; ++i) {
      t[i] = b * kCoefBlock + i < K
                 ? fma(blk[2 * kCoefBlock + i], yn2, fma(blk[kCoefBlock + i], yn, blk[i]))
                 : -INFINITY;
      mx = fmax(mx, t[i]);
    }
    nlive += (unsigned)min(kCoefBlock, K - b * kCoefBlock);
    const double mn = fmax(a.m, ceil(mx));
    a.s = ldexp(a.s, (int)fmax(a.m - mn, -2100.0));
    a.m = mn;
    const double ms = mn == -INFINITY ? 0.0 : mn;
    double sum = 0.0;
#pragma unroll
    for (int i = 0; i < kCoefBlock; ++i) sum += exp2(t[i] - ms);
    a.s += sum;
  }
  acc[l][j] = a;
  if (census && j == 0 && nlive) atomicAdd(&live_n, nlive);
  TabAcc ce{-INFINITY, 0.0}, cg{-INFINITY, 0.0};
  for (int k = tid; k < K; k += kTabThreads) {
    const double x = cf[coef_off(k, 0)], y = cf[coef_off(k, 1)], z = cf[coef_off(k, 2)];
    const double ak = -z, mu = y / (2.0 * ak), cc = x + ak * mu * mu;
    const double d = fmax(0.0, fmax(pl - mu, mu - ph)), df = fmax(mu - pl, ph - mu);
    tab_add(ce, cc + 8.0 * log2(2.0 * ak / L2E) - 0.5 * ak * d * d);
    tab_add(cg, cc - ak * df * df);
  }
  ce = tab_wave_sum(ce);
  cg = tab_wave_sum(cg);
  if ((tid & 63) == 0) { cert[0][tid >> 6] = ce; cert[1][tid >> 6] = cg; }
  __syncthreads();
  double nm = -INFINITY, ns = 0.0;
  if (tid < kTabNodes) {
    TabAcc v = acc[0][tid];
    for (int q = 1; q < 16; ++q) tab_merge(v, acc[q][tid]);
    nm = v.m;
    ns = v.s;
    double M = nm;
#pragma unroll
    for (int o = 8; o > 0; o >>= 1) M = fmax(M, __shfl_xor(M, o, 64));
    fn[tid] = ldexp(ns, (int)fmax(nm - (M == -INFINITY ? 0.0 : M), -2100.0));
    if (tid == 0) red[0] = M;
  }
  __syncthreads();
  const double M = red[0];
  if (tid < kTabNodes) {
    double c = 0.0;
    for (int q = 0; q < kTabNodes; ++q)
      c = fma(fn[q], cospi((double)(tid * (2 * q + 1)) / 32.0), c);
    c *= tid == 0 ? 1.0 / 16.0 : 2.0 / 16.0;
    cn[tid] = c;
    tab[(int64_t)slot * kTabMaxPanels + p].c[tid] = c;
  }
  __syncthreads();
  if (tid != 0) return;
  tab[(int64_t)slot * kTabMaxPanels + p].M = M;
  tab[(int64_t)slot * kTabMaxPanels + p].pad = 0.0;
  if (census) {
    atomicAdd(census + 3, (unsigned long long)kTabNodes * (unsigned long long)K);
    atomicAdd(census + 5, (unsigned long long)kTabNodes * (unsigned long long)live_n);
  }
  bool ok = M > -INFINITY && M < INFINITY;
  double ca = 0.0;
  for (int q = 0; q < kTabNodes; ++q) {
    ok = ok && fn[q] > 0.0 && fn[q] < INFINITY;
    ca += fabs(cn[q]);
  }
  TabAcc E = cert[0][0], G = cert[1][0];
  for (int q = 1; q < 4; ++q) { tab_merge(E, cert[0][q]); tab_merge(G, cert[1][q]); }
  const double kL16 = 44.25014046988262;
  const double le = 0.11960158 + 0.5 * kL16 + (E.m + log2(E.s)) + 16.0 * log2(Hh) - 15.0 - kL16;
  const double lr = M + log2(ca) - 46.0;
  const double lg = G.m + log2(G.s);
  ok = ok && le == le && le < INFINITY && lg > -INFINITY && lg < INFINITY &&
       fmax(le, lr) + 1.0 <= lg - 28.0;
  if (ok) atomicAdd(&hdr[slot].ncert, 1u);
}

constexpr int kBndThreads = 256;
constexpr double kBndWiden = 0x1p-20;
constexpr int kBndPieces = 8;
static_assert(kBndCells % kBndThreads == 0 && kBndCells >= 2 * kTabMaxPanels, "lattice shape");

struct BndSide {
  double va, vb;
  double lo;
  double d1, d2;
  double e;
  double M;
};
__device__ __forceinline__ BndSide bound_side(const TabHdr &h, const TabPanel *__restrict__ tab,
                                              double xa, double xb) {
  const double um = (0.5 * (xa + xb) - h.y_lo) * h.inv_w;
  const double pf = fmin(fmax(floor(um), 0.0), (double)(h.P - 1));
  const TabPanel &pn = tab[(int)pf];
  double c[kTabNodes];
#pragma unroll
  for (int k = 0; k < kTabNodes; ++k) c[k] = pn.c[k];
  const double ta = fmin(fmax(2.0 * ((xa - h.y_lo) * h.inv_w - pf) - 1.0, -1.0), 1.0);
  const double tb = fmin(fmax(2.0 * ((xb - h.y_lo) * h.inv_w - pf) - 1.0, -1.0), 1.0);
  double s0 = 0.0, s1 = 0.0, s2 = 0.0;
#pragma unroll
  for (int k = 0; k < kTabNodes; ++k) {
    const double a = fabs(c[k]), k2 = (double)(k * k);
    s0 += a;
    s1 += k2 * a;
    s2 += k2 * (k2 - 1.0) / 3.0 * a;
  }
  BndSide r;
  r.va = tab_clenshaw(c, ta);
  r.vb = tab_clenshaw(c, tb);
  r.d1 = s1 * (2.0 * h.inv_w);
  r.d2 = s2 * (4.0 * h.inv_w * h.inv_w);
  r.e = s0 * 0x1p-46 + s1 * 0x1p-40;
  const double hh = xb - xa;
  r.lo = fmin(r.va, r.vb) - hh * hh * 0.125 * r.d2 - r.e;
  r.M = pn.M;
  return r;
}
__device__ __forceinline__ double bound_next_edge(const TabHdr &h, double x) {
  const double w = 1.0 / h.inv_w;
  const double j = floor((x - h.y_lo) * h.inv_w) + 1.0;
  const double e = h.y_lo + j * w;
  return e > x ? e : h.y_lo + (j + 1.0) * w;
}

__global__ __launch_bounds__(kBndThreads) void k_table_bound(
    const tpe_hp *__restrict__ hps, const TabHdr *__restrict__ hdr,
    const TabPanel *__restrict__ tab, double *__restrict__ bound) {
  const int hp = blockIdx.y, cell = blockIdx.x * kBndThreads + threadIdx.x;
  const tpe_hp H = hps[hp];
  if (!table_hp(H)) return;
  const TabHdr hb = hdr[2 * (int64_t)hp], ha = hdr[2 * (int64_t)hp + 1];
  if (!(tab_valid(hb) && tab_valid(ha))) return;
  const TabPanel *__restrict__ tb = tab + 2 * (int64_t)hp * kTabMaxPanels;
  const TabPanel *__restrict__ ta = tb + kTabMaxPanels;
  const double LN2 = 0.6931471805599453;
  const double y_lo = H.low - H.prior_mu, y_hi = H.high - H.prior_mu;
  const double cw = (y_hi - y_lo) / (double)kBndCells;
  const double a0 = cell == 0 ? y_lo : fmax(y_lo, y_lo + cw * ((double)cell - kBndWiden));
  const double b0 =
      cell == kBndCells - 1 ? y_hi : fmin(y_hi, y_lo + cw * ((double)(cell + 1) + kBndWiden));
  double U = -INFINITY, x = a0;
  bool ok = a0 < b0;
  for (int it = 0; it < kBndPieces && ok && x < b0; ++it) {
    const double nx = fmin(b0, fmin(bound_next_edge(hb, x), bound_next_edge(ha, x)));
    const BndSide B = bound_side(hb, tb, x, nx), A = bound_side(ha, ta, x, nx);
    const double la = log2(B.va / A.va), lb = log2(B.vb / A.vb), dm = B.M - A.M;
    const double sa = (dm + la) * LN2, sb = (dm + lb) * LN2;
    const double gb = B.d1 / B.lo, ga = A.d1 / A.lo;
    const double curv = B.d2 / B.lo + gb * gb + A.d2 / A.lo + ga * ga;
    const double slack =
        2.0 * (B.e / B.lo + A.e / A.lo) + 0x1p-40 * (1.0 + fabs(dm) + fabs(la) + fabs(lb));
    const double hh = nx - x;
    const double u = fmax(sa, sb) + hh * hh * 0.125 * curv + slack;
    ok = B.lo > 0.0 && A.lo > 0.0 && sa == sa && sb == sb && u == u && u < INFINITY;
    U = fmax(U, u);
    x = nx;
  }
  ok = ok && !(x < b0);
  bound[(int64_t)hp * kBndCells + cell] = ok ? U : INFINITY;
}

hipError_t launch_table_build(const tpe_hp *hps, int32_t n_hp, const MixInfo *info,
                              const Coef *coef, int64_t kcap, TabHdr *hdr, TabPanel *tab,
                              unsigned long long *census, hipStream_t st, double *bound) {
  if (n_hp <= 0) return hipSuccess;
  hipError_t e = hipMemsetAsync(hdr, 0, (size_t)2 * n_hp * sizeof(TabHdr), st);
  if (e != hipSuccess) return e;
  k_table_build<<<dim3(kTabMaxPanels, 2 * n_hp), kTabThreads, 0, st>>>(hps, info, coef, kcap, hdr,
                                                                       tab, census);
  if (bound)
    k_table_bound<<<dim3(kBndCells / kBndThreads, n_hp), kBndThreads, 0, st>>>(hps, hdr, tab, bound);
  return hipGetLastError();
}

}
```

### hyperopt_amd/csrc/tpe_level_plan.hpp

```cpp
#pragma once
#include <algorithm>
#include <cstdint>
#include <utility>
#include <vector>

#include "tpe_internal.hpp"
#include "tpe_switches.hpp"

namespace tpe {

constexpr int64_t kSortedDrawMin = (int64_t)1 << 22;
constexpr int64_t kSmallSortMin = 2048;
constexpr int64_t kTileDrawMax = 4096;

inline int32_t active_bound(const std::vector<tpe_hp> &all, const std::vector<int32_t> &cond_parent,
                            const std::vector<int32_t> &cond_branch, const int32_t *hps, int b,
                            int e) {
  int32_t n = 0;
  std::vector<std::pair<int32_t, int32_t>> pb;
  for (int i = b; i < e; ++i) {
    const tpe_hp &x = all[hps[i]];
    if (x.cond_count == 0) { ++n; continue; }
    std::vector<std::pair<int32_t, int32_t>> mine;
    for (int c = 0; c < x.cond_count; ++c)
// ... 47 lines not shown
        const int k = score_kind(hps[hp]);
        L.kinds.push_back(k);
        if (k == KIND_CAT) L.cat_upper = std::max<int64_t>(L.cat_upper, hps[hp].upper);
        L.table_slot |= (k == KIND_LSE_G || k == KIND_LSE_L) && table_hp(hps[hp]);
      }
      while (L.n_lat < n && (L.kinds[L.n_lat] == KIND_ERF_G || L.kinds[L.n_lat] == KIND_ERF_L) &&
             lat[hl[L.n_lat]].R > 0) {
        L.rmax = std::max<int64_t>(L.rmax, lat[hl[L.n_lat]].R);
        ++L.n_lat;
      }
      auto bound = [&](int b, int e) {
        return active_bound(hps, cond_parent, cond_branch, hl.data(), b, e);
      };
      L.rows_level = bound(0, n);
      L.rows_lead = bound(0, L.n_lat);
      L.rows_plain.assign(n, 0);
      L.rows_lat.assign(n, 0);
      for (int with_lat = 0; with_lat < 2; ++with_lat) {
        auto kind = [&](int i) { return with_lat && i < L.n_lat ? (int)KIND_LAT : L.kinds[i]; };
        for (int j = 0; j < n;) {
          int k = j;
          while (k < n && kind(k) == kind(j)) ++k;
          (with_lat ? L.rows_lat : L.rows_plain)[j] = bound(j, k);
          j = k;
        }
      }
    }
  }
};

enum { BELOW_FUSE = 0,
       BELOW_TABLE = 1,
       BELOW_LARGE = 2 };
inline int below_class(int64_t k) {
  return k <= kFuseTab ? BELOW_FUSE : k <= kTabCap ? BELOW_TABLE : BELOW_LARGE;
}

struct FitVariant {
  bool small = false;
  int32_t mom_w = 0;
  bool mom_h = false;
  bool operator==(const FitVariant &o) const {
    return small == o.small && mom_w == o.mom_w && mom_h == o.mom_h;
  }
};

inline int32_t mom_width(const PlanShape &ps, const Switches &sw, int64_t n_hist) {
  if (!sw.moment) return 0;
  double kmax = 0.0;
  for (size_t i = 0; i < ps.hps.size(); ++i) {
    const int k = score_kind(ps.hps[i]);
    if (k == KIND_LSE_G || k == KIND_LSE_L) kmax = std::max(kmax, (double)n_hist * ps.act_frac[i]);
  }
  if (kmax >= (double)kMom16MinK) return 16;
  if (kmax >= (double)sw.lse_shift_min) return 8;
  return 0;
}

inline bool step_reads_moments(const PlanShape &ps, int64_t n_sug, int64_t n_cand) {
  bool sorted = false;
  for (const auto &l : ps.levels) sorted |= n_cand * n_sug * (int64_t)l.size() >= kSortedDrawMin;
  return sorted && n_cand > kWaveRowSplitMax;
}

inline FitVariant fit_variant(const PlanShape &ps, const Switches &sw, int64_t n_hist, bool small,
                              bool moments) {
  FitVariant f;
  f.small = small;
  f.mom_w = moments ? mom_width(ps, sw, n_hist) : 0;
  f.mom_h = f.mom_w == 16;
  return f;
}

struct StepShape {
  int64_t n_sug = 0, n_cand = 0, cand_begin = 0;
  int64_t n_total = 0;
  int32_t below = BELOW_LARGE;
  FitVariant fit;
  int32_t prune_mode = 3;
  bool lattice_on = true;
  bool capturing = false;
  bool publish = false;
  int32_t screen_run = 0;
  bool operator==(const StepShape &o) const {
    return n_sug == o.n_sug && n_cand == o.n_cand && cand_begin == o.cand_begin &&
           n_total == o.n_total && below == o.below && fit == o.fit &&
           prune_mode == o.prune_mode && lattice_on == o.lattice_on &&
           capturing == o.capturing && publish == o.publish && screen_run == o.screen_run;
  }
};
inline int32_t step_screen_run(const Switches &sw) {
  return sw.draw_screen && sw.draw_screen_int ? (int32_t)sw.draw_screen_run : 0;
}

struct ScoreGrid {
  int32_t n_groups = 0, pstride = 1;
  int32_t grp_kind[kMaxGroups] = {}, grp_slot0[kMaxGroups] = {}, grp_tiles[kMaxGroups] = {};
  int32_t grp_block0[kMaxGroups + 1] = {}, grp_slots[kMaxGroups] = {};
  int32_t blocks() const { return grp_block0[n_groups]; }
};
template <typename Kind, typename Rows>
ScoreGrid score_grid(Kind kind, int n_slots, int64_t cn, Rows rows) {
  ScoreGrid g;
  int32_t blocks = 0;
  auto weight = [](int k) {
    if (k == KIND_ERF_G || k == KIND_ERF_L) return 0;
    if (kind_lse(k)) return 1;
    return k == KIND_LAT ? 2 : 3;
  };
  for (int pass = 0; pass < 4; ++pass) {
    for (int j = 0; j < n_slots;) {
      int k = j;
      while (k < n_slots && kind(k) == kind(j)) ++k;
      if (weight(kind(j)) != pass) { j = k; continue; }
      if (g.n_groups == kMaxGroups) { g.pstride = -1; return g; }
      const int i = g.n_groups++;
      const int64_t tc = tile_cands(kind(j));
      const int32_t nt = (int32_t)((std::max<int64_t>(cn, 0) + tc - 1) / tc);
      g.grp_kind[i] = kind(j);
      g.grp_slot0[i] = j;
      g.grp_slots[i] = k - j;
      g.grp_tiles[i] = nt;
      g.grp_block0[i] = blocks;
      blocks += nt * std::min<int32_t>(k - j, rows(j, k));
      g.pstride = std::max(g.pstride, nt);
      j = k;
    }
  }
  g.grp_block0[g.n_groups] = blocks;
  return g;
}

inline int grid_classes(const ScoreGrid &g, bool lookup_draw) {
  int m = 0;
  for (int i = 0; i < g.n_groups; ++i) {
    const int k = g.grp_kind[i];
    m |= 1 << (kind_wave_lse(k) ? 0 : lookup_draw && (k == KIND_CAT || k == KIND_LAT) ? 1 : 2);
  }
  return m;
}

enum class LatRun {
  None,
  InOrder,
  Side,
  Deferred,
  Fused,
};

enum class Draw {
  Tiles,
  Fused,
  Plain,
  Sorted,
  SortedPruned,
  SortedScreened,
};

struct ChunkPlan {
  int64_t c0 = 0, cn = 0;
  bool accumulate = false;
  ScoreGrid grid;
  int32_t sort_log2 = 0, lse_pos = 0, lse_prune = 0, lse_f32 = 0, lookup_draw = 0;
  bool lk_fork = false;
  Draw draw = Draw::Plain;
  bool table_draw = false;
  bool small_table = false;
  bool fast = false;
  int32_t screen_tiles = 0;
  int32_t screen_guide = -1;
  int32_t screen_run = 0;
// ... 145 lines not shown
```

### hyperopt_amd/csrc/tpe_score.hip

```cpp
#include <math.h>

#include <algorithm>
#include <cstdlib>
#include <type_traits>

#include "tpe_device.hpp"
#include "tpe_draw.hpp"
#include "tpe_lpdf.hpp"
#include "tpe_switches.hpp"

namespace tpe {

constexpr int kWaves = 8;
constexpr int kRMax = 2;
constexpr int kChunk = 16;
static_assert(2 * kRMax <= kWaves, "one merging wave per (mixture, candidate row)");


typedef uint64_t __attribute__((address_space(1))) gu64;
typedef uint32_t __attribute__((address_space(1))) gu32;
__device__ __forceinline__ uint64_t dbits(double x) { return __builtin_bit_cast(uint64_t, x); }
__device__ __forceinline__ double bitsd(uint64_t x) { return __builtin_bit_cast(double, x); }


// ... 2270 lines not shown
  const int ntl = min(kMapTiles, nt - tile0);
  double x[kMapTiles][KR];
#pragma unroll
  for (int j = 0; j < kMapTiles; ++j)
    if (j < ntl) table_wave_load(A, s, slot, logn, (tile0 + j) * kWaves + wave, x[j]);
  double *__restrict__ wmax = A.tab_wmax + ((int64_t)s * A.n_hp + hp) * A.pstride * kWaves;
#pragma unroll
  for (int j = 0; j < kMapTiles; ++j) {
    if (j >= ntl) break;
    const int wt = (tile0 + j) * kWaves + wave;
    const double best = table_wave_tile<CENSUS, true>(A, s, hp, logn, wt, mu, x[j]);
    if ((threadIdx.x & 63) == 0) wmax[wt] = best;
  }
}

constexpr int kMapDpTiles = 512;
__host__ __device__ inline int table_map_dp_blocks(const ScoreArgs &A, int g) {
  const int rows = (A.grp_block0[g + 1] - A.grp_block0[g]) / A.grp_tiles[g];
  return rows * ((A.grp_tiles[g] * kWaves + kMapDpTiles - 1) / kMapDpTiles);
}
template <bool CENSUS>
__global__ __launch_bounds__(kWaves * 64) void k_table_map_dp(ScoreArgs A) {
  constexpr int KR = kMapRows, PW = kMapDpTiles / kWaves;
  static_assert(PW == 64, "a wave's tile mask: one entry per lane");
  const int b = blockIdx.x;
  int g = 0, b0 = 0;
  for (; g + 1 < A.n_groups; ++g) {
    const int nb = table_map_dp_blocks(A, g);
    if (b < b0 + nb) break;
    b0 += nb;
  }
  const int ntw = A.grp_tiles[g] * kWaves, nsb = (ntw + kMapDpTiles - 1) / kMapDpTiles;
  const int local = b - b0;
  int slot = A.grp_slot0[g] + local / nsb;
  const int s = blockIdx.y;
  if (A.compact) {
    slot = active_slot(A, s, A.grp_slot0[g], A.grp_slots[g], local / nsb);
    if (slot < 0) return;
  }
  const int hp = A.level_hps[slot];
  const int64_t sb = 2 * (int64_t)hp, sa = sb + 1;
  if (!(tab_valid(A.tab_hdr[sb]) && tab_valid(A.tab_hdr[sa]))) return;
  if (!(A.force_active || A.compact ||
        hp_active(A.hps[hp], A.results + (int64_t)s * A.n_hp, A.cond_parent, A.cond_branch)))
    return;
  const bool logn = A.grp_kind[g] == KIND_LSE_LW;
  const double mu = A.hps[hp].prior_mu;
  const int wave = __builtin_amdgcn_readfirstlane((int)(threadIdx.x >> 6));
  const int lane = threadIdx.x & 63;
  double *__restrict__ wmax = A.tab_wmax + ((int64_t)s * A.n_hp + hp) * A.pstride * kWaves;
  const int wt0 = (local % nsb) * kMapDpTiles + wave;
  const int wl = wt0 + kWaves * lane;
  const bool in = wl < ntw;
  const bool drop = in && (int64_t)wl * (64 * KR) < A.n_cand && wmax[wl] == -INFINITY;
  auto uniform64 = [](uint64_t m) {
    return ((uint64_t)(uint32_t)__builtin_amdgcn_readfirstlane((int)(uint32_t)(m >> 32)) << 32) |
           (uint32_t)__builtin_amdgcn_readfirstlane((int)(uint32_t)m);
  };
  uint64_t todo = uniform64(__ballot(in && !drop));
  if constexpr (CENSUS) {
    uint64_t dr = uniform64(__ballot(drop));
    while (dr) {
      const int wt = wt0 + kWaves * (int)__builtin_ctzll(dr);
      dr &= dr - 1;
      if (lane == 0) {
        const unsigned long long c =
            (unsigned long long)min<int64_t>(64 * KR, A.n_cand - (int64_t)wt * (64 * KR)) *
            (unsigned long long)(A.info[sb].K + A.info[sa].K);
        atomicAdd(A.census + 3, c);
        atomicAdd(A.census + 12, c);
      }
    }
  }
  while (todo) {
    const int wt = wt0 + kWaves * (int)__builtin_ctzll(todo);
    todo &= todo - 1;
    double x[KR];
    table_wave_load(A, s, slot, logn, wt, x);
    const double best = table_wave_tile<CENSUS, true>(A, s, hp, logn, wt, mu, x);
    if (lane == 0) wmax[wt] = best;
  }
}

constexpr int kPilotThreads = 1024;
__global__ __launch_bounds__(kPilotThreads) void k_table_pilot(ScoreArgs A) {
  constexpr int NW = kPilotThreads / 64;
  constexpr int WC = 64 * tile_rows(KIND_LSE_GW);
  constexpr int NWORD = kBndCells / 64;
  static_assert(kBndCells % kPilotThreads == 0 && kPilotWaves % NW == 0, "pilot shape");
  __shared__ double wsc[kPilotWaves];
  __shared__ unsigned long long hotw[NWORD];
  const int s = blockIdx.y, tid = threadIdx.x, lane = tid & 63;
  const int wave = __builtin_amdgcn_readfirstlane(tid >> 6);
  int row = blockIdx.x;
  const int g = row_group(A, row);
  int slot = A.grp_slot0[g] + row;
  if (A.compact) {
    slot = active_slot(A, s, A.grp_slot0[g], A.grp_slots[g], row);
    if (slot < 0) return;
  }
  const int hp = A.level_hps[slot];
  if (!(tab_valid(A.tab_hdr[2 * (int64_t)hp]) && tab_valid(A.tab_hdr[2 * (int64_t)hp + 1]))) return;
  if (!(A.force_active || A.compact ||
        hp_active(A.hps[hp], A.results + (int64_t)s * A.n_hp, A.cond_parent, A.cond_branch)))
    return;
  const int np = (int)min<int64_t>(min(kPilotWaves, A.grp_tiles[g] * kWaves), (A.n_cand + WC - 1) / WC);
  const bool logn = A.grp_kind[g] == KIND_LSE_LW;
  const double mu = A.hps[hp].prior_mu;
  for (int wt = wave; wt < np; wt += NW) {
    double x[kMapRows];
    table_wave_load(A, s, slot, logn, wt, x);
    const double v = table_wave_tile<false, false>(A, s, hp, logn, wt, mu, x);
    if (lane == 0) wsc[wt] = v;
  }
  __syncthreads();
  double L0 = np > 0 ? -INFINITY : NAN;
  for (int i = 0; i < np; ++i) {
    const double v = wsc[i];
    L0 = (v != v || L0 != L0) ? NAN : fmax(L0, v);
  }
  const double T0 = L0 - A.tab_tie * fmax(1.0, fabs(L0));
  const bool all = !(L0 == L0) || fabs(L0) == INFINITY;
  const double *__restrict__ U = A.tab_bound + (int64_t)hp * kBndCells;
  for (int c0 = 0; c0 < kBndCells; c0 += kPilotThreads) {
    const uint64_t bal = __ballot(all || !(U[c0 + tid] < T0));
    if (lane == 0) hotw[(c0 + tid) >> 6] = bal;
  }
  __syncthreads();
  if (tid != 0) return;
  const tpe_hp H = A.hps[hp];
  const double y_lo = H.low - H.prior_mu, y_hi = H.high - H.prior_mu;
  const double cw = (y_hi - y_lo) / (double)kBndCells;
  int r0[kHotIv + 1], r1[kHotIv + 1], n = 0;
  auto next_cell = [&](int c, bool hot) {
    while (c < kBndCells) {
      const unsigned long long w = (hot ? hotw[c >> 6] : ~hotw[c >> 6]) >> (c & 63);
      if (w) return c + (int)__builtin_ctzll(w);
      c = (c | 63) + 1;
    }
    return (int)kBndCells;
  };
  for (int c = next_cell(0, true); c < kBndCells;) {
    const int e = next_cell(c, false);
    const int a0 = max(c - 1, 0), a1 = min(e, kBndCells - 1);
    if (n > 0 && a0 <= r1[n - 1] + 1) {
      r1[n - 1] = a1;
    } else {
      r0[n] = a0;
      r1[n] = a1;
      if (++n > kHotIv) {
        int bj = 1, bg = r0[1] - r1[0];
        for (int j = 2; j < n; ++j)
          if (r0[j] - r1[j - 1] < bg) { bg = r0[j] - r1[j - 1]; bj = j; }
        r1[bj - 1] = r1[bj];
        for (int j = bj; j + 1 < n; ++j) { r0[j] = r0[j + 1]; r1[j] = r1[j + 1]; }
        --n;
      }
    }
    c = next_cell(e, true);
  }
  TabHot *out = A.tab_hot + ((int64_t)s * A.n_hp + hp);
  out->y_lo = y_lo;
  out->y_hi = y_hi;
  for (int i = 0; i < kHotIv; ++i) {
    const bool on = i < n;
    out->lo[i] = !on ? INFINITY : r0[i] == 0 ? -INFINITY : y_lo + cw * (double)r0[i];
// ... 20 lines not shown
      for (int i = tid; i < A.grp_slots[g]; i += 64) {
        const int hp = A.level_hps[A.grp_slot0[g] + i];
        if (!hp_active(A.hps[hp], res, A.cond_parent, A.cond_branch)) {
          res[hp] = Partial{NAN, NAN, -1, 0, 0};
          A.tie_cnt[(int64_t)s * A.n_hp + hp] = 0;
        }
      }
    }
    slot = active_slot(A, s, A.grp_slot0[g], A.grp_slots[g], row);
    if (slot < 0) return;
  }
  const int hp = A.level_hps[slot];
  const int64_t sh = (int64_t)s * A.n_hp + hp;
  const bool act = A.force_active || A.compact ||
                   hp_active(A.hps[hp], A.results + (int64_t)s * A.n_hp, A.cond_parent,
                             A.cond_branch);
  if (!act) {
    if (tid == 0) {
      A.results[sh] = Partial{NAN, NAN, -1, 0, 0};
      A.tie_cnt[sh] = 0;
    }
    return;
  }
  const int ntw = nt * kWaves;
  int32_t *list = A.tie_list + sh * A.pstride * kWaves;
  if (!(tab_valid(A.tab_hdr[2 * (int64_t)hp]) && tab_valid(A.tab_hdr[2 * (int64_t)hp + 1]))) {
    const int SBB = (1 << A.sort_log2) / tile_cands(KIND_LSE_GW);
    for (int e = tid; e < ntw; e += kGatherThreads) {
      const int j = e / kWaves, w = e % kWaves;
      const int sb = j / SBB, q = j % SBB;
      const int nbs = min(SBB, nt - sb * SBB);
      list[e] = sb * SBB * kWaves + q + nbs * w;
    }
    if (tid == 0) A.tie_cnt[sh] = ntw;
    return;
  }
  const double *wm = A.tab_wmax + sh * A.pstride * kWaves;
  const int nrec = (int)min<int64_t>(ntw, (A.n_cand + WC - 1) / WC);
  double m = -INFINITY;
  int nan = 0;
  for (int i = tid; i < nrec; i += kGatherThreads) {
    const double v = wm[i];
    nan |= v != v;
    m = fmax(m, v);
  }
#pragma unroll
  for (int o = 32; o > 0; o >>= 1) {
    m = fmax(m, __shfl_xor(m, o, 64));
    nan |= __shfl_xor(nan, o, 64);
  }
  if (lane == 0) { red_s[wave] = m; red_n[wave] = nan; }
  __syncthreads();
  m = red_s[0];
  nan = red_n[0];
#pragma unroll
  for (int w = 1; w < NW; ++w) { m = fmax(m, red_s[w]); nan |= red_n[w]; }
  const double tm = (nan || nrec <= 0) ? NAN : m;
  if (tid == 0) A.tab_max[sh] = tm;
  const double wthr = tm - A.tab_tie * fmax(1.0, fabs(tm));
  const bool dp = A.tab_pref == 2;
  int base = 0;
  for (int i0 = 0; i0 < ntw; i0 += kGatherThreads) {
    const int i = i0 + tid;
    const bool hot = i < ntw && !(wm[i] < wthr) && !(dp && i < nrec && wm[i] == -INFINITY);
    const uint64_t bal = __ballot(hot);
    if (lane == 0) wsum[wave] = __popcll(bal);
    __syncthreads();
    int before = 0, total = 0;
#pragma unroll
    for (int w = 0; w < NW; ++w) {
      const int c = wsum[w];
      before += w < wave ? c : 0;
      total += c;
    }
    if (hot) list[base + before + __popcll(bal & (((uint64_t)1 << lane) - 1))] = i;
    base += total;
    __syncthreads();
  }
  if (tid == 0) {
    A.tie_cnt[sh] = base;
    if (base == 0 && !A.accumulate) A.results[sh] = Partial{NAN, NAN, -1, 1, 0};
  }
}
template <bool CENSUS, int MW>
__global__ __launch_bounds__(kWaves * 64) __attribute__((amdgpu_waves_per_eu(TPE_WAVE_EU)))
void k_score_wave1(ScoreArgs A) {
  __shared__ ScoreSmem1 sm;
  score_block<kSetWave1, CENSUS, ScoreSmem1, MW>(A, sm);
}

template <bool CENSUS>
__global__ __launch_bounds__(kWaves * 64) __attribute__((amdgpu_waves_per_eu(4)))
void k_score_tdraw(ScoreArgs A) {
  __shared__ ScoreSmem sm;
  score_block<kSetTiny, CENSUS>(A, sm);
}

template <bool CENSUS>
__global__ __launch_bounds__(kWaves * 64) __attribute__((amdgpu_waves_per_eu(4)))
void k_score_lookup(ScoreArgs A) {
  __shared__ ScoreSmemT<1> sm;
  score_block<kSetLookup, CENSUS>(A, sm);
}

template <int I>
struct RowShlSum {
  static __device__ __forceinline__ double run(double pc, double v) {
    static_assert(I < 16, "row_shl reaches 15 lanes");
    return RowShlSum<I - 1>::run(pc, v) + dppd<0x100 + I>(v);
  }
};
template <>
struct RowShlSum<0> {
  static __device__ __forceinline__ double run(double pc, double) { return pc; }
};

template <bool LOGN>
__device__ __forceinline__ void lattice_point(const ScoreArgs &A, const tpe_hp &H, int hp,
                                              const LatInfo &L, int64_t pt, double *csum,
                                              double2 *__restrict__ out) {
#pragma clang fp contract(off)
  const double x = (double)(L.j0 + pt) * H.q;
  double ub, lb;
  quant_bounds<LOGN>(H, x, ub, lb);
  const int64_t sb = 2 * (int64_t)hp;
  const MixInfo ib = A.info[sb], ia = A.info[sb + 1];
  const int ncb = (ib.K + kChunk - 1) / kChunk, nca = (ia.K + kChunk - 1) / kChunk;
  const int nch = ncb + nca;
  const double *cb = reinterpret_cast<const double *>(A.coef + sb * A.kcap);
  const double *ca = reinterpret_cast<const double *>(A.coef + (sb + 1) * A.kcap);
  const int j = threadIdx.x & (kChunk - 1);
  constexpr int kLatU = 4;
  for (int t0 = 0; t0 < kChunk * nch; t0 += kLatU * (int)blockDim.x) {
    double cx[kLatU], cy[kLatU], cw[kLatU];
    bool ok[kLatU];
#pragma unroll
    for (int u = 0; u < kLatU; ++u) {
      const int c = (t0 + u * (int)blockDim.x + (int)threadIdx.x) / kChunk;
      const bool above = c >= ncb;
      const int k = (above ? c - ncb : c) * kChunk + j;
      ok[u] = c < nch && k < (above ? ia.K : ib.K);
      const double *cs = above ? ca : cb;
      cx[u] = ok[u] ? cs[coef_off(k, 0)] : 0.0;
      cy[u] = ok[u] ? cs[coef_off(k, 1)] : 0.0;
      cw[u] = ok[u] ? cs[coef_off(k, 2)] : 0.0;
    }
#pragma unroll
    for (int u = 0; u < kLatU; ++u) {
      const int c = (t0 + u * (int)blockDim.x + (int)threadIdx.x) / kChunk;
      double inc = 0.0;
      if (ok[u]) {
        const double zu = (ub - cx[u]) * cy[u], zl = (lb - cx[u]) * cy[u];
        if (!erf_dead(zu, zl)) inc = erf_term<LOGN>(zu, zl, cw[u]);
      }
      const double pc = RowShlSum<kChunk - 1>::run(0.0 + inc, inc);
      if (j == 0 && c < nch) csum[c] = pc;
    }
  }
  __syncthreads();
  const int t = threadIdx.x;
  double sw = 0.0;
  if (t < 2 * kWaves) {
    const int above = t / kWaves, w = t % kWaves;
    const int c0 = above ? ncb : 0, n = above ? nca : ncb;
    for (int c = w; c < n; c += kWaves) sw += csum[c0 + c];
  }
// ... 62 lines not shown
    LatJobs J{};
    int64_t rmax = 0;
    const int32_t n = std::min<int32_t>(kLatJobs, n_lat - i0);
    for (int32_t i = 0; i < n; ++i) {
      const int32_t hp = hps_of_level[i0 + i];
      J.job[i].H = hps[hp];
      J.job[i].L = lat[hp];
      J.job[i].hp = hp;
      rmax = std::max<int64_t>(rmax, lat[hp].R);
    }
    if (rmax > kLatMaxR) return hipErrorInvalidValue;
    if (rmax <= 0) continue;
    J.n_jobs = n;
    k_lattice<false><<<dim3((unsigned)rmax, (unsigned)n), kLatThreads,
                       (size_t)nch * sizeof(double), st>>>(a, J, lat_out);
    const hipError_t e = hipGetLastError();
    if (e != hipSuccess) return e;
  }
  return hipSuccess;
}

const void *lattice_draw_kernel_fn() { return reinterpret_cast<const void *>(&k_lattice<true>); }

hipError_t launch_lattice_draw(const ScoreArgs &a, const int32_t *hps_of_level, const tpe_hp *hps,
                               const LatInfo *lat, int32_t n_lat, double2 *lat_out,
                               hipStream_t st, int32_t lat_rows) {
  static_assert(kLatThreads == 256, "draw rows run k_draw's 256-thread blocks");
  const int64_t nch = 2 * ((a.kcap + kChunk - 1) / kChunk);
  if (nch > kLatChunks || n_lat < 1 || n_lat > kLatJobs || a.n_cand <= 0) return hipErrorInvalidValue;
  LatJobs J{};
  int64_t rmax = 0;
  for (int32_t i = 0; i < n_lat; ++i) {
    const int32_t hp = hps_of_level[i];
    J.job[i].H = hps[hp];
    J.job[i].L = lat[hp];
    J.job[i].hp = hp;
    rmax = std::max<int64_t>(rmax, lat[hp].R);
  }
  if (rmax > kLatMaxR || rmax <= 0) return hipErrorInvalidValue;
  const int64_t gx = (a.n_cand + kLatThreads - 1) / kLatThreads;
  const int64_t draws = gx * a.slot_rows * a.n_suggest;
  if (draws > ((int64_t)1 << 30)) return hipErrorInvalidValue;
  J.n_jobs = n_lat;
  if (lat_rows > 0 && lat_rows < n_lat) {
    J.n_jobs = lat_rows;
    J.compact = 1;
    J.n_lat = n_lat;
  }
  J.draw_gx = (int32_t)gx;
  J.draw_blocks = (int32_t)draws;
  const int64_t rows = (draws + rmax - 1) / rmax;
  const size_t lds = std::max<size_t>((size_t)nch * sizeof(double), sizeof(DrawTableT<kFuseTab>));
  k_lattice<true><<<dim3((unsigned)rmax, (unsigned)(J.n_jobs + rows)), kLatThreads, lds, st>>>(
      a, J, lat_out);
  return hipGetLastError();
}

static int group_class(const ScoreArgs &a, int kind) {
  if (kind_wave_lse(kind)) return 0;
  if (a.lookup_draw && (kind == KIND_CAT || kind == KIND_LAT)) return 1;
  return 2;
}
static ScoreArgs select_groups(const ScoreArgs &a, int cls) {
  ScoreArgs b = a;
  b.n_groups = 0;
  int32_t blocks = 0;
  for (int i = 0; i < a.n_groups; ++i) {
    if (group_class(a, a.grp_kind[i]) != cls) continue;
    const int j = b.n_groups++;
    b.grp_kind[j] = a.grp_kind[i];
    b.grp_slot0[j] = a.grp_slot0[i];
    b.grp_tiles[j] = a.grp_tiles[i];
    b.grp_slots[j] = a.grp_slots[i];
    b.grp_block0[j] = blocks;
    blocks += a.grp_block0[i + 1] - a.grp_block0[i];
  }
  b.grp_block0[b.n_groups] = blocks;
  return b;
}

constexpr int kTieBlocksPerCu = 16;

static bool table_scalar_on() { return switches().table_scalar; }

static hipError_t launch_class(const ScoreArgs &a, int cls, bool has_erf, hipStream_t st) {
  if (a.n_groups <= 0) return hipSuccess;
  const int blocks = a.grp_block0[a.n_groups];
  if (blocks <= 0) return hipSuccess;
  const dim3 g((unsigned)blocks, a.n_suggest);
  bool one_row = false;
  for (int i = 0; i < a.n_groups; ++i)
    one_row |= a.grp_kind[i] == KIND_LSE_GW1 || a.grp_kind[i] == KIND_LSE_LW1;
  const bool m8 = a.lse_mom == 8;
  if (cls == 0 && one_row) {
    if (m8) {
      if (a.census) k_score_wave1<true, 8><<<g, kWaves * 64, 0, st>>>(a);
      else k_score_wave1<false, 8><<<g, kWaves * 64, 0, st>>>(a);
    } else {
      if (a.census) k_score_wave1<true, 16><<<g, kWaves * 64, 0, st>>>(a);
      else k_score_wave1<false, 16><<<g, kWaves * 64, 0, st>>>(a);
    }
  } else if (cls == 0) {
    if (a.tab_on == 2) {
      if (table_scalar_on()) {
        if (a.census) k_score_table<true, false, true><<<g, kWaves * 64, 0, st>>>(a);
        else k_score_table<false, false, true><<<g, kWaves * 64, 0, st>>>(a);
      } else {
        if (a.census) k_score_table<true><<<g, kWaves * 64, 0, st>>>(a);
        else k_score_table<false><<<g, kWaves * 64, 0, st>>>(a);
      }
      return hipGetLastError();
    }
    if (a.tab_on) {
      if (!a.tie_list || !a.tie_cnt) return hipErrorInvalidValue;
      int32_t rows = 0, ntmax = 1;
      for (int i = 0; i < a.n_groups; ++i) {
        rows += (a.grp_block0[i + 1] - a.grp_block0[i]) / a.grp_tiles[i];
        ntmax = std::max(ntmax, a.grp_tiles[i]);
      }
      if (rows <= 0 || rows > 65535 || a.n_suggest > 65535) return hipErrorInvalidValue;
      if (a.tab_pref == 1) {
        if (!a.tab_bound || !a.tab_hot) return hipErrorInvalidValue;
        k_table_pilot<<<dim3((unsigned)rows, a.n_suggest), kPilotThreads, 0, st>>>(a);
      }
      if (table_scalar_on() && a.tab_pref == 2) {
        int32_t mb = 0;
        for (int i = 0; i < a.n_groups; ++i) mb += table_map_dp_blocks(a, i);
        const dim3 gm((unsigned)mb, a.n_suggest);
        if (a.census) k_table_map_dp<true><<<gm, kWaves * 64, 0, st>>>(a);
        else k_table_map_dp<false><<<gm, kWaves * 64, 0, st>>>(a);
      } else if (table_scalar_on()) {
        int32_t mb = 0;
        for (int i = 0; i < a.n_groups; ++i) mb += table_map_blocks(a, i);
        const dim3 gm((unsigned)mb, a.n_suggest);
        if (a.census) k_table_map<true><<<gm, kWaves * 64, 0, st>>>(a);
        else k_table_map<false><<<gm, kWaves * 64, 0, st>>>(a);
      } else {
        if (a.census) k_score_table<true, true><<<g, kWaves * 64, 0, st>>>(a);
        else k_score_table<false, true><<<g, kWaves * 64, 0, st>>>(a);
      }
      k_tie_gather<<<dim3((unsigned)rows, a.n_suggest), kGatherThreads, 0, st>>>(a);
      const int64_t per = ((int64_t)kTieBlocksPerCu * kNumCUs + (int64_t)rows * a.n_suggest - 1) /
                          ((int64_t)rows * a.n_suggest);
      const unsigned G = (unsigned)std::max<int64_t>(1, std::min<int64_t>(ntmax, per));
      const dim3 gt(G, (unsigned)rows, a.n_suggest);
      if (a.census) k_score_wave_tie<true><<<gt, kWaves * 64, 0, st>>>(a);
      else k_score_wave_tie<false><<<gt, kWaves * 64, 0, st>>>(a);
      return hipGetLastError();
    }
    if (m8) {
      if (a.census) k_score_wave<true, 8><<<g, kWaves * 64, 0, st>>>(a);
      else k_score_wave<false, 8><<<g, kWaves * 64, 0, st>>>(a);
    } else {
      if (a.census) k_score_wave<true, 16><<<g, kWaves * 64, 0, st>>>(a);
      else k_score_wave<false, 16><<<g, kWaves * 64, 0, st>>>(a);
    }
  } else if (cls == 1) {
    ScoreArgs b = a;
    int64_t rows_all = 0;
    for (int i = 0; i < a.n_groups; ++i)
      rows_all += (a.grp_block0[i + 1] - a.grp_block0[i]) / a.grp_tiles[i];
    const int64_t pieces = (a.n_cand + 2047) / 2048;
    const int64_t want = std::max<int64_t>(1, (4 * kNumCUs) / std::max<int64_t>(1, rows_all * a.n_suggest));
    const int64_t nseg0 = std::min<int64_t>(pieces, want);
    b.lookup_seg = (pieces + nseg0 - 1) / nseg0 * 2048;
    const int32_t nseg = (int32_t)((a.n_cand + b.lookup_seg - 1) / b.lookup_seg);
    int32_t blk = 0;
    for (int i = 0; i < b.n_groups; ++i) {
      const int32_t rows = (a.grp_block0[i + 1] - a.grp_block0[i]) / a.grp_tiles[i];
      b.grp_block0[i] = blk;
      b.grp_tiles[i] = nseg;
      blk += rows * nseg;
    }
    b.grp_block0[b.n_groups] = blk;
    const dim3 gl((unsigned)blk, a.n_suggest);
    if (b.census) k_score_lookup<true><<<gl, kWaves * 64, 0, st>>>(b);
    else k_score_lookup<false><<<gl, kWaves * 64, 0, st>>>(b);
  } else if (has_erf) {
    if (a.census) k_score<true, true><<<g, kWaves * 64, 0, st>>>(a);
    else k_score<true, false><<<g, kWaves * 64, 0, st>>>(a);
  } else {
    if (a.census) k_score<false, true><<<g, kWaves * 64, 0, st>>>(a);
    else k_score<false, false><<<g, kWaves * 64, 0, st>>>(a);
  }
  return hipGetLastError();
}

hipError_t launch_table_pilot(const ScoreArgs &a0, hipStream_t st) {
  const ScoreArgs a = score_classes(a0) == 1 ? a0 : select_groups(a0, 0);
  if (a.n_groups <= 0 || !a.tab_bound || !a.tab_hot) return hipErrorInvalidValue;
  int32_t rows = 0;
  for (int i = 0; i < a.n_groups; ++i)
    rows += (a.grp_block0[i + 1] - a.grp_block0[i]) / a.grp_tiles[i];
  if (rows <= 0 || rows > 65535 || a.n_suggest > 65535) return hipErrorInvalidValue;
  k_table_pilot<<<dim3((unsigned)rows, a.n_suggest), kPilotThreads, 0, st>>>(a);
  return hipGetLastError();
}

int score_classes(const ScoreArgs &a) {
  int m = 0;
  for (int i = 0; i < a.n_groups; ++i) m |= 1 << group_class(a, a.grp_kind[i]);
  return m;
}

hipError_t launch_score(const ScoreArgs &a, bool has_erf, hipStream_t st, hipStream_t side,
                        hipEvent_t ev_fork, hipEvent_t ev_join, int classes) {
  if (a.n_groups <= 0 || a.n_suggest <= 0) return hipSuccess;
  if (a.grp_block0[a.n_groups] <= 0) return hipSuccess;
  if (a.tile_draw) {
    const dim3 g((unsigned)a.grp_block0[a.n_groups], a.n_suggest);
    if (a.census) k_score_tdraw<true><<<g, kWaves * 64, 0, st>>>(a);
    else k_score_tdraw<false><<<g, kWaves * 64, 0, st>>>(a);
    return hipGetLastError();
  }
  bool has[3] = {false, false, false};
  for (int i = 0; i < a.n_groups; ++i) has[group_class(a, a.grp_kind[i])] = true;
  for (int c = 0; c < 3; ++c) has[c] = has[c] && ((classes >> c) & 1);
  const int ncls = (int)has[0] + (int)has[1] + (int)has[2];
  if (ncls == 0) return hipSuccess;
  if (ncls == 1) {
    const int c = has[0] ? 0 : has[1] ? 1 : 2;
    return launch_class(score_classes(a) == (1 << c) ? a : select_groups(a, c), c, has_erf, st);
  }
  hipError_t e;
// ... 17 lines not shown
```

### hyperopt_amd/csrc/tpe_switches.hpp

```cpp
#pragma once
#include <cmath>
#include <cstdint>
#include <cstdlib>

#include "tpe_internal.hpp"

namespace tpe {

struct Switches {
  bool lookup_draw;
  bool lookup_fork;
  bool publish;
  bool tile_draw;
  bool publish_fuse;
  bool moment;
  bool table;
  bool draw_prune;
  bool draw_screen;
  bool draw_screen_int;
  bool table_prefilter;
  bool table_scalar;
  bool small_sort;
  bool side_streams;
  bool graph;
  int64_t table_tie_log2;
  int64_t draw_screen_tiles;
  int64_t draw_screen_min;
  int64_t draw_screen_guide_bits;
  int64_t draw_screen_run;
  int64_t chunk_mb;
  int64_t lse_shift_min;

  double table_tie() const { return std::ldexp(1.0, (int)table_tie_log2); }
  int64_t chunk_budget() const { return chunk_mb << 17; }
};

constexpr int64_t kDrawScreenMin = (int64_t)1 << 26;
constexpr int64_t kDrawScreenRun = 4;

enum class SwitchRule {
  OffIfZero,
  OffIfNonEmptyZero,
  OnIfNonZero,
  OnIfSet,
  ValueIfSet,
  ValueIfNonEmpty,
};

struct SwitchDef {
  const char *name;
  SwitchRule rule;
  int64_t dflt;
  bool Switches::*flag;
  int64_t Switches::*value;
  int64_t lo, hi;
};

constexpr int64_t kTabTieLog2 = -16;
static_assert(kTabTie == 0x1p-16, "kTabTie is 2^kTabTieLog2");

inline const SwitchDef *switch_table(int *n) {
  using R = SwitchRule;
  using S = Switches;
  constexpr int64_t lo = INT64_MIN, hi = INT64_MAX;
  static const SwitchDef defs[] = {
      {"TPE_LOOKUP_DRAW", R::OffIfZero, 1, &S::lookup_draw, nullptr, 0, 0},
      {"TPE_LOOKUP_FORK", R::OffIfZero, 1, &S::lookup_fork, nullptr, 0, 0},
      {"TPE_PUBLISH", R::OffIfZero, 1, &S::publish, nullptr, 0, 0},
      {"TPE_TILE_DRAW", R::OffIfZero, 1, &S::tile_draw, nullptr, 0, 0},
      {"TPE_PUBLISH_FUSE", R::OffIfZero, 1, &S::publish_fuse, nullptr, 0, 0},
      {"TPE_MOMENT", R::OffIfZero, 1, &S::moment, nullptr, 0, 0},
      {"TPE_TABLE", R::OffIfZero, 1, &S::table, nullptr, 0, 0},
      {"TPE_DRAW_PRUNE", R::OffIfNonEmptyZero, 1, &S::draw_prune, nullptr, 0, 0},
      {"TPE_DRAW_SCREEN", R::OffIfNonEmptyZero, 1, &S::draw_screen, nullptr, 0, 0},
      {"TPE_DRAW_SCREEN_INT", R::OffIfNonEmptyZero, 1, &S::draw_screen_int, nullptr, 0, 0},
      {"TPE_TABLE_PREFILTER", R::OffIfNonEmptyZero, 1, &S::table_prefilter, nullptr, 0, 0},
      {"TPE_TABLE_SCALAR", R::OffIfNonEmptyZero, 1, &S::table_scalar, nullptr, 0, 0},
      {"TPE_SMALL_SORT", R::OnIfNonZero, 0, &S::small_sort, nullptr, 0, 0},
      {"TPE_SIDE_STREAMS", R::OnIfSet, 0, &S::side_streams, nullptr, 0, 0},
      {"TPE_GRAPH", R::OnIfSet, 0, &S::graph, nullptr, 0, 0},
      {"TPE_TABLE_TIE_LOG2", R::ValueIfSet, kTabTieLog2, nullptr, &S::table_tie_log2, -1074, 4096},
      {"TPE_DRAW_SCREEN_TILES", R::ValueIfNonEmpty, 2, nullptr, &S::draw_screen_tiles, 0,
       kPilotWaves},
      {"TPE_DRAW_SCREEN_MIN", R::ValueIfNonEmpty, kDrawScreenMin, nullptr, &S::draw_screen_min, lo,
       hi},
      {"TPE_DRAW_SCREEN_GUIDE_BITS", R::ValueIfNonEmpty, 9, nullptr, &S::draw_screen_guide_bits, 0,
       kGuideBitsMax},
      {"TPE_DRAW_SCREEN_RUN", R::ValueIfNonEmpty, kDrawScreenRun, nullptr, &S::draw_screen_run, 0,
       kScreenRunMax},
      {"TPE_CHUNK_MB", R::ValueIfSet, 8192, nullptr, &S::chunk_mb, lo, hi},
      {"TPE_SHIFT_MIN_K", R::ValueIfSet, 512, nullptr, &S::lse_shift_min, lo, hi},
  };
  *n = (int)(sizeof(defs) / sizeof(defs[0]));
  return defs;
}

template <typename Get>
Switches read_switches(Get get) {
  Switches s{};
  int n = 0;
  const SwitchDef *defs = switch_table(&n);
  for (int i = 0; i < n; ++i) {
    const SwitchDef &d = defs[i];
    const char *e = get(d.name);
    switch (d.rule) {
      case SwitchRule::OffIfZero: s.*d.flag = !(e && std::atoi(e) == 0); break;
      case SwitchRule::OffIfNonEmptyZero: s.*d.flag = !(e && *e && std::atoi(e) == 0); break;
      case SwitchRule::OnIfNonZero: s.*d.flag = e && std::atoi(e) != 0; break;
      case SwitchRule::OnIfSet: s.*d.flag = e != nullptr; break;
      case SwitchRule::ValueIfSet:
      case SwitchRule::ValueIfNonEmpty: {
        const bool set = e && (d.rule == SwitchRule::ValueIfSet || *e);
        const int64_t v = set ? (int64_t)std::atoll(e) : d.dflt;
        s.*d.value = v < d.lo ? d.lo : v > d.hi ? d.hi : v;
        break;
      }
    }
  }
  return s;
}

inline const Switches &switches() {
  static const Switches s = read_switches([](const char *name) { return std::getenv(name); });
  return s;
}

}
```

### include/tpe_engine.h

```cpp
#ifndef TPE_ENGINE_H
#define TPE_ENGINE_H

#include <stdint.h>

#ifdef __cplusplus
extern "C" {
#endif

#define TPE_ENGINE_ABI_VERSION 1

#define TPE_SHARD_ALIGN 8192

#define TPE_OK 0
#define TPE_E_INVALID (-1)
#define TPE_E_BOUNDS (-2)
#define TPE_E_NEGATIVE (-3)
#define TPE_E_NOMEM (-4)
#define TPE_E_HIP (-5)
#define TPE_E_NODEVICE (-6)
#define TPE_E_INDEX (-7)

#define TPE_GMM 0
#define TPE_LGMM 1
#define TPE_CAT 2
// ... 122 lines not shown

int tpe_plan_score_candidates(tpe_plan_t p, int32_t hp, const double *x,
                              int64_t n, double *llik_b, double *llik_a,
                              int64_t *best_index, double *best_score);

int tpe_plan_score_candidates_sorted(tpe_plan_t p, int32_t hp, int32_t mode,
                                     const double *x, int64_t n, double *llik_b,
                                     double *llik_a, int64_t *best_index,
                                     double *best_score);

int tpe_plan_score_points(tpe_plan_t p, const double *vals, int64_t m, int64_t ld,
                          double *total, double *terms, uint8_t *active,
                          int32_t on_device, void *stream);

int tpe_plan_sample_points(tpe_plan_t p, uint64_t seed, int64_t begin, int64_t m,
                           int64_t ld, double *vals, double *total, double *terms,
                           uint8_t *active, int32_t on_device, void *stream);

int tpe_plan_topk_points(tpe_plan_t p, const double *total, const uint8_t *eligible,
                         int64_t m, int32_t k, int32_t *idx, int32_t on_device,
                         void *stream);

int tpe_plan_gather_points(tpe_plan_t p, const double *vals, int64_t ld,
                           const int32_t *idx, int32_t k, double *out,
                           int32_t on_device, void *stream);

int tpe_plan_joint_fit(tpe_plan_t p, void *stream);
int tpe_plan_joint_get_mixture(tpe_plan_t p, int32_t hp, int32_t side, double *w,
                               double *mu, double *sigma, int32_t *rows, int64_t cap,
                               int64_t *k);
int tpe_plan_joint_score_points(tpe_plan_t p, const double *vals, int64_t m, int64_t ld,
                                double *total, double *joint, double *terms,
                                uint8_t *active, int32_t on_device, void *stream);
int tpe_plan_joint_sides(tpe_plan_t p, double *below, double *above, int64_t m);
int tpe_plan_joint_sample_points(tpe_plan_t p, uint64_t seed, int64_t begin, int64_t m,
                                 int64_t ld, double *vals, int32_t *comp, double *total,
                                 double *joint, double *terms, uint8_t *active,
                                 int32_t on_device, void *stream);

int tpe_plan_group_info(tpe_plan_t p, int32_t *group_of_hp, int32_t *n_groups);
int tpe_plan_group_fit(tpe_plan_t p, void *stream);
int tpe_plan_group_get_mixture(tpe_plan_t p, int32_t group, int32_t hp, int32_t side,
                               double *w, double *mu, double *sigma, int32_t *rows,
                               int64_t cap, int64_t *k);
int tpe_plan_group_score_points(tpe_plan_t p, const double *vals, int64_t m, int64_t ld,
                                double *total, double *joint, uint8_t *active,
                                int32_t on_device, void *stream);
int tpe_plan_group_sides(tpe_plan_t p, int32_t group, double *below, double *above,
                         int64_t m);
int tpe_plan_group_sample_points(tpe_plan_t p, uint64_t seed, int64_t begin, int64_t m,
                                 int64_t ld, double *vals, int32_t *comp, double *total,
                                 double *joint, uint8_t *active, int32_t on_device,
                                 void *stream);

int tpe_plan_group_batch_points(tpe_plan_t p, const double *vals, int64_t m, int64_t ld,
                                const uint8_t *eligible, int32_t k, int32_t *idx,
                                double *gain, double *trace, int32_t on_device,
                                void *stream);

#define TPE_MAX_OBJ 8
int tpe_plan_set_objectives(tpe_plan_t p, const double *Y, int32_t n_obj, int64_t n,
                            int64_t ld, int64_t obj0, int32_t on_device, void *stream);

int tpe_plan_pareto_get(tpe_plan_t p, int32_t *dominated_by, int32_t *dominates,
                        double *loss, int64_t n);

int tpe_plan_pareto_shape(tpe_plan_t p, int64_t n, int32_t n_obj, int64_t force_splits,
                          int64_t *out);

int tpe_plan_last_stats(tpe_plan_t p, double *score_ms, double *pairs);

int tpe_plan_profile(tpe_plan_t p, int32_t capacity);
int tpe_plan_profile_read(tpe_plan_t p, int32_t kind, double *avg_ms,
                          int64_t *launches, double *pairs_per_launch);

int tpe_plan_set_lattice(tpe_plan_t p, int32_t enable);

int tpe_plan_census(tpe_plan_t p, int32_t enable, int64_t *counts);
int tpe_plan_census_n(tpe_plan_t p, int32_t enable, int64_t *counts, int32_t n_counts);

int tpe_plan_tie_counts(tpe_plan_t p, int32_t n_suggest, int32_t *counts);
int tpe_plan_tab_wmax(tpe_plan_t p, int32_t n_suggest, double *out);
int tpe_plan_tab_bound(tpe_plan_t p, int32_t hp, double *out);
int tpe_plan_tab_hot(tpe_plan_t p, int32_t n_suggest, double *out);
int64_t tpe_plan_cand_dump(tpe_plan_t p, int32_t s, int32_t hp, double *values,
                           int32_t *positions);
int tpe_plan_draw_screen_stats(tpe_plan_t p, int64_t *out);

int tpe_plan_sample_prior(tpe_plan_t p, const uint64_t *seeds, int64_t n_suggest,
                          tpe_result *out, int32_t out_on_device, void *stream);

int tpe_plan_set_anneal_order(tpe_plan_t p, const int32_t *hp_order, int32_t n_hp);
int tpe_plan_anneal(tpe_plan_t p, double avg_best_idx, double shrink_coef,
                    const uint64_t *seeds, int64_t n_suggest,
                    tpe_result *out, int32_t out_on_device, void *stream);

typedef struct { int32_t row; int32_t rank; double u[4]; } tpe_anneal_trace;
int tpe_plan_anneal_trace(tpe_plan_t p, int32_t n_suggest, tpe_anneal_trace *out);

int tpe_plan_set_prune(tpe_plan_t p, int32_t mode);

int tpe_microbench(tpe_handle_t h, int32_t which, double *per_second);

int tpe_math_probe(tpe_handle_t h, int32_t which, const double *x, int64_t n, double *out);

#ifdef __cplusplus
}
#endif
#endif
```

Measured before the change: 1211000 billion pairs/s.

## Add lean table build with precomputed mixture terms and skip-negligible LSE adds

```diff
diff --git a/hyperopt_amd/_engine.py b/hyperopt_amd/_engine.py
--- a/hyperopt_amd/_engine.py
+++ b/hyperopt_amd/_engine.py
@@ -36,6 +36,7 @@
     'tpe_plan_sample_prior', 'tpe_plan_score_candidates_sorted', 'tpe_plan_census_n',
     'tpe_plan_tie_counts', 'tpe_plan_tab_wmax', 'tpe_plan_anneal', 'tpe_plan_anneal_trace',
     'tpe_plan_set_anneal_order', 'tpe_plan_tab_bound', 'tpe_plan_tab_hot',
+    'tpe_plan_tab_panels', 'tpe_plan_tab_cert', 'tpe_plan_tie_list',
     'tpe_plan_cand_dump', 'tpe_plan_draw_screen_stats', 'tpe_plan_score_points',
     'tpe_plan_sample_points', 'tpe_plan_topk_points', 'tpe_plan_gather_points',
     'tpe_plan_joint_fit', 'tpe_plan_joint_get_mixture', 'tpe_plan_joint_score_points',
@@ -180,6 +181,9 @@
             'tpe_plan_tab_wmax': (C.c_int, [vp, i32, vp]),
             'tpe_plan_tab_bound': (C.c_int, [vp, i32, vp]),
             'tpe_plan_tab_hot': (C.c_int, [vp, i32, vp]),
+            'tpe_plan_tab_panels': (C.c_int, [vp, i32, i32, vp, vp, vp, vp]),
+            'tpe_plan_tab_cert': (C.c_int, [vp, i32, i32, vp]),
+            'tpe_plan_tie_list': (C.c_int, [vp, i32, i32, vp]),
             'tpe_plan_cand_dump': (C.c_int64, [vp, i32, i32, vp, vp]),
             'tpe_plan_draw_screen_stats': (C.c_int, [vp, vp]),
             'tpe_plan_set_lattice': (C.c_int, [vp, i32]),
@@ -1006,6 +1010,35 @@
             e.check(e.lib.tpe_plan_tab_bound(self.p, int(hp), out.ctypes.data))
         return out
 
+    def tab_panels(self, hp, side):
+        e = self.engine
+        y_lo, inv_w, ncert = C.c_double(), C.c_double(), C.c_int32()
+        buf = np.zeros((64, 144), dtype=np.uint8)
+        with e.lock:
+            n = e.lib.tpe_plan_tab_panels(self.p, int(hp), int(side), C.addressof(y_lo),
+                                          C.addressof(inv_w), C.addressof(ncert), buf.ctypes.data)
+            e.check(min(n, 0))
+        return dict(y_lo=y_lo.value, inv_w=inv_w.value, P=int(n), ncert=int(ncert.value),
+                    panels=buf[:n].copy())
+
+    def tab_cert(self, hp, side):
+        e = self.engine
+        out = np.zeros((64, 3), dtype=np.float64)
+        with e.lock:
+            n = e.lib.tpe_plan_tab_cert(self.p, int(hp), int(side), out.ctypes.data)
+            e.check(min(n, 0))
+        return out[:n].copy()
+
+    def tie_list(self, s, hp):
+        e = self.engine
+        with e.lock:
+            n = e.lib.tpe_plan_tie_list(self.p, int(s), int(hp), None)
+            e.check(min(n, 0))
+            out = np.empty(n, dtype=np.int32)
+            if n:
+                e.check(min(e.lib.tpe_plan_tie_list(self.p, int(s), int(hp), out.ctypes.data), 0))
+        return out
+
     def tab_hot(self, n_suggest):
         e = self.engine
         out = np.empty((int(n_suggest), self.n_hp, 18), dtype=np.float64)
diff --git a/hyperopt_amd/csrc/tpe_engine.hip b/hyperopt_amd/csrc/tpe_engine.hip
--- a/hyperopt_amd/csrc/tpe_engine.hip
+++ b/hyperopt_amd/csrc/tpe_engine.hip
@@ -58,6 +58,8 @@
   int32_t *d_tie_cnt = nullptr;
   int32_t tab_pstride = 0;
   double *d_tab_bound = nullptr;
+  double *d_tab_terms = nullptr;
+  double *d_tab_cert = nullptr;
   TabHot *d_tab_hot = nullptr;
   DrawZone *d_draw_zone = nullptr;
   unsigned long long *d_screen_stats = nullptr;
@@ -244,6 +246,7 @@
                   p->d_ticket, p->d_sortbuf, p->d_census, p->d_lat_info, p->d_lat, p->d_coef32, p->d_coefm,
                   p->d_coefm8, p->d_coefe, p->d_coefmh, p->d_tab_hdr, p->d_tab,
                   p->d_tab_max, p->d_tab_wmax, p->d_tie_list, p->d_tie_cnt, p->d_tab_bound,
+                  p->d_tab_terms, p->d_tab_cert,
                   p->d_tab_hot, p->d_draw_zone, p->d_screen_stats, p->d_pt_vals, p->d_pt_terms,
                   p->d_pt_total, p->d_pt_act, p->d_pt_idx, p->d_pt_count, p->d_pt_tab, p->d_tk,
                   p->d_tk_idx, p->d_jdims, p->d_jdim_of_hp, p->d_jrows, p->d_jcount, p->d_jcomp,
@@ -422,6 +425,7 @@
   CKH(hipMemset(p->d_tab_hdr, 0, (size_t)slots * sizeof(TabHdr)));
   CKH(dalloc(&p->d_tab, (size_t)slots * kTabMaxPanels));
   CKH(dalloc(&p->d_tab_bound, (size_t)p->P * kBndCells));
+  if (switches().table_lean) CKH(dalloc(&p->d_tab_terms, table_terms_doubles(p->P, kcap)));
   p->act_frac.assign(p->P, 1.0);
   for (const auto &lv : p->levels)
     for (int i : lv) {
@@ -674,7 +678,8 @@
   if (p->tab_built) return TPE_OK;
   CKH(launch_table_build(p->d_hps, p->P, p->d_info, p->d_coef, p->kcap, p->d_tab_hdr, p->d_tab,
                          p->census ? p->d_census : nullptr, st,
-                         switches().table_prefilter ? p->d_tab_bound : nullptr));
+                         switches().table_prefilter ? p->d_tab_bound : nullptr, p->d_tab_terms,
+                         p->d_tab_cert));
   p->tab_built = true;
   return TPE_OK;
 }
@@ -714,6 +719,7 @@
   s.prune_mode = p->prune_mode;
   s.lattice_on = p->lattice_on;
   s.screen_run = step_screen_run(switches());
+  s.table_lean = switches().table_lean;
   return s;
 }
 
@@ -3095,6 +3101,77 @@
   return TPE_OK;
 }
 
+static int tab_header(tpe_plan *p, int32_t hp, int32_t side, TabHdr *th) {
+  tpe_engine *h = p->eng;
+  if (hp < 0 || hp >= p->P || side < 0 || side > 1) return fail(h, TPE_E_INVALID, "bad args");
+  if (!table_hp(p->hps[hp])) return fail(h, TPE_E_INVALID, "hp has no Chebyshev table");
+  CKH(hipSetDevice(h->device));
+  CKH(hipDeviceSynchronize());
+  const int rc = table_build(h, p, h->stream);
+  if (rc) return rc;
+  CKH(hipMemcpyAsync(th, p->d_tab_hdr + 2 * (int64_t)hp + side, sizeof(*th), hipMemcpyDeviceToHost,
+                     h->stream));
+  CKH(hipStreamSynchronize(h->stream));
+  if (th->P < 0 || th->P > kTabMaxPanels) return fail(h, TPE_E_HIP, "table header out of range");
+  return TPE_OK;
+}
+
+int tpe_plan_tab_panels(tpe_plan_t p, int32_t hp, int32_t side, double *y_lo, double *inv_w,
+                        int32_t *ncert, void *panels) {
+  if (!p) return TPE_E_INVALID;
+  tpe_engine *h = p->eng;
+  TabHdr th;
+  const int rc = tab_header(p, hp, side, &th);
+  if (rc) return rc;
+  if (y_lo) *y_lo = th.y_lo;
+  if (inv_w) *inv_w = th.inv_w;
+  if (ncert) *ncert = (int32_t)th.ncert;
+  if (panels && th.P > 0)
+    CKH(hipMemcpy(panels, p->d_tab + (2 * (int64_t)hp + side) * kTabMaxPanels,
+                  (size_t)th.P * sizeof(TabPanel), hipMemcpyDeviceToHost));
+  return th.P;
+}
+
+int tpe_plan_tab_cert(tpe_plan_t p, int32_t hp, int32_t side, double *out) {
+  if (!p) return TPE_E_INVALID;
+  tpe_engine *h = p->eng;
+  if (!p->d_tab_cert) {
+    CKH(hipSetDevice(h->device));
+    CKH(hipDeviceSynchronize());
+    graph_reset(p);
+    const size_t n = (size_t)2 * p->P * kTabMaxPanels * 3;
+    CKH(dalloc(&p->d_tab_cert, n));
+    CKH(hipMemset(p->d_tab_cert, 0xff, n * sizeof(double)));
+    p->tab_built = false;
+  }
+  TabHdr th;
+  const int rc = tab_header(p, hp, side, &th);
+  if (rc) return rc;
+  if (out && th.P > 0)
+    CKH(hipMemcpy(out, p->d_tab_cert + (2 * (int64_t)hp + side) * kTabMaxPanels * 3,
+                  (size_t)th.P * 3 * sizeof(double), hipMemcpyDeviceToHost));
+  return th.P;
+}
+
+int tpe_plan_tie_list(tpe_plan_t p, int32_t s, int32_t hp, int32_t *out) {
+  if (!p) return TPE_E_INVALID;
+  tpe_engine *h = p->eng;
+  if (hp < 0 || hp >= p->P || s < 0 || s >= p->s_cap || p->tab_pstride <= 0 ||
+      ((size_t)s * p->P + hp + 1) * p->tab_pstride > p->partial_cap)
+    return fail(h, TPE_E_INVALID, "hp / suggestion not of the last launch that took the tables");
+  CKH(hipSetDevice(h->device));
+  CKH(hipDeviceSynchronize());
+  int32_t n = 0;
+  CKH(hipMemcpy(&n, p->d_tie_cnt + (int64_t)s * p->P + hp, sizeof(n), hipMemcpyDeviceToHost));
+  const int64_t row = (int64_t)p->tab_pstride * 8;
+  if (n < 0) return 0;
+  if (n > row) return fail(h, TPE_E_HIP, "tie count out of range");
+  if (out && n > 0)
+    CKH(hipMemcpy(out, p->d_tie_list + ((int64_t)s * p->P + hp) * row, (size_t)n * sizeof(int32_t),
+                  hipMemcpyDeviceToHost));
+  return n;
+}
+
 int tpe_plan_draw_screen_stats(tpe_plan_t p, int64_t *out) {
   if (!p || !out) return TPE_E_INVALID;
   tpe_engine *h = p->eng;
diff --git a/hyperopt_amd/csrc/tpe_internal.hpp b/hyperopt_amd/csrc/tpe_internal.hpp
--- a/hyperopt_amd/csrc/tpe_internal.hpp
+++ b/hyperopt_amd/csrc/tpe_internal.hpp
@@ -374,9 +374,14 @@
 
 hipError_t launch_micro(int which, int blocks, int iters, double *sink, hipStream_t st);
 hipError_t launch_math_probe(int which, const double *x, int64_t n, double *out, hipStream_t st);
+constexpr int kTabTermDoubles = 4;
+inline size_t table_terms_doubles(int32_t n_hp, int64_t kcap) {
+  return (size_t)2 * n_hp * ((size_t)kcap * kTabTermDoubles + 1);
+}
 hipError_t launch_table_build(const tpe_hp *hps, int32_t n_hp, const MixInfo *info,
                               const Coef *coef, int64_t kcap, TabHdr *hdr, TabPanel *tab,
-                              unsigned long long *census, hipStream_t st, double *bound = nullptr);
+                              unsigned long long *census, hipStream_t st, double *bound = nullptr,
+                              double *terms = nullptr, double *cert = nullptr);
 
 constexpr int kPatchVals = 192;
 constexpr int kPatchLoss = 16;
diff --git a/hyperopt_amd/csrc/tpe_kernels.hip b/hyperopt_amd/csrc/tpe_kernels.hip
--- a/hyperopt_amd/csrc/tpe_kernels.hip
+++ b/hyperopt_amd/csrc/tpe_kernels.hip
@@ -4,6 +4,7 @@
 #include <cstdlib>
 
 #include "tpe_draw.hpp"
+#include "tpe_tab_add.hpp"
 
 namespace tpe {
 
@@ -715,15 +716,6 @@
 constexpr int kTabThreads = 256;
 constexpr double kTabSkip = 64.0;
 
-struct TabAcc {
-  double m, s;
-};
-__device__ __forceinline__ void tab_add(TabAcc &a, double t) {
-  const double mn = fmax(a.m, ceil(t));
-  a.s = ldexp(a.s, (int)fmax(a.m - mn, -2100.0));
-  a.m = mn;
-  a.s += exp2(t - (mn == -INFINITY ? 0.0 : mn));
-}
 __device__ __forceinline__ void tab_merge(TabAcc &a, const TabAcc &b) {
   const double M = fmax(a.m, b.m);
   const double ms = M == -INFINITY ? 0.0 : M;
@@ -739,10 +731,66 @@
   return a;
 }
 
-__global__ __launch_bounds__(kTabThreads) void k_table_build(
+struct __attribute__((aligned(32))) TabTerm {
+  double mu;
+  double cc;
+  double Ak;
+  double ak;
+};
+constexpr double kTabL2E = 1.4426950408889634;
+#pragma clang fp contract(off)
+__device__ __forceinline__ TabTerm tab_term(double x, double y, double z) {
+  TabTerm t;
+  t.ak = -z;
+  t.mu = y / (2.0 * t.ak);
+  t.cc = __builtin_fma(t.ak * t.mu, t.mu, x);
+  t.Ak = t.cc + 8.0 * log2(2.0 * t.ak / kTabL2E);
+  return t;
+}
+__device__ __forceinline__ void tab_cert_terms(const TabTerm &t, double pl, double ph, double &te,
+                                               double &tg) {
+  const double d = fmax(0.0, fmax(pl - t.mu, t.mu - ph)), df = fmax(t.mu - pl, ph - t.mu);
+  te = __builtin_fma(-((0.5 * t.ak) * d), d, t.Ak);
+  tg = __builtin_fma(-(t.ak * df), df, t.cc);
+}
+#pragma clang fp contract(fast)
+
+__global__ __launch_bounds__(kTabThreads) void k_table_terms(
+    const tpe_hp *__restrict__ hps, const MixInfo *__restrict__ info,
+    const Coef *__restrict__ coef, int64_t kcap, TabTerm *__restrict__ terms,
+    double *__restrict__ a2s) {
+  const int slot = blockIdx.y, tid = threadIdx.x, k = blockIdx.x * kTabThreads + tid;
+  if (!table_hp(hps[slot >> 1])) return;
+  const int K = info[slot].K;
+  if (K < 1 || K > kcap) return;
+  const double *__restrict__ cf = reinterpret_cast<const double *>(coef + (int64_t)slot * kcap);
+  if (k < K)
+    terms[(int64_t)slot * kcap + k] =
+        tab_term(cf[coef_off(k, 0)], cf[coef_off(k, 1)], cf[coef_off(k, 2)]);
+  if (blockIdx.x != 0) return;
+  __shared__ double red[4];
+  double a2 = 0.0;
+  for (int k0 = tid; k0 < K; k0 += 4 * kTabThreads) {
+    double z[4];
+#pragma unroll
+    for (int j = 0; j < 4; ++j) z[j] = cf[coef_off(min(k0 + j * kTabThreads, K - 1), 2)];
+#pragma unroll
+    for (int j = 0; j < 4; ++j) a2 = fmax(a2, -z[j]);
+  }
+#pragma unroll
+  for (int o = 32; o > 0; o >>= 1) a2 = fmax(a2, __shfl_xor(a2, o, 64));
+  if ((tid & 63) == 0) red[tid >> 6] = a2;
+  __syncthreads();
+  if (tid == 0) a2s[slot] = fmax(fmax(red[0], red[1]), fmax(red[2], red[3]));
+}
+
+template <bool LEAN>
+__device__ __forceinline__ void table_build_body(
     const tpe_hp *__restrict__ hps, const MixInfo *__restrict__ info,
     const Coef *__restrict__ coef, int64_t kcap, TabHdr *__restrict__ hdr,
-    TabPanel *__restrict__ tab, unsigned long long *__restrict__ census) {
+    TabPanel *__restrict__ tab, unsigned long long *__restrict__ census,
+    const TabTerm *__restrict__ terms, const double *__restrict__ a2s,
+    double *__restrict__ cert_out) {
   const int slot = blockIdx.y, p = blockIdx.x, tid = threadIdx.x;
   const tpe_hp H = hps[slot >> 1];
   if (!table_hp(H)) return;
@@ -756,13 +804,19 @@
   __shared__ double fn[kTabNodes], cn[kTabNodes];
   __shared__ unsigned live_n;
   double a2 = 0.0;
-  for (int k = tid; k < K; k += kTabThreads) a2 = fmax(a2, -cf[coef_off(k, 2)]);
-#pragma unroll
-  for (int o = 32; o > 0; o >>= 1) a2 = fmax(a2, __shfl_xor(a2, o, 64));
-  if ((tid & 63) == 0) red[tid >> 6] = a2;
-  if (tid == 0) live_n = 0u;
-  __syncthreads();
-  a2 = fmax(fmax(red[0], red[1]), fmax(red[2], red[3]));
+  if constexpr (LEAN) {
+    if (tid == 0) live_n = 0u;
+    __syncthreads();
+    a2 = a2s[slot];
+  } else {
+    for (int k = tid; k < K; k += kTabThreads) a2 = fmax(a2, -cf[coef_off(k, 2)]);
+#pragma unroll
+    for (int o = 32; o > 0; o >>= 1) a2 = fmax(a2, __shfl_xor(a2, o, 64));
+    if ((tid & 63) == 0) red[tid >> 6] = a2;
+    if (tid == 0) live_n = 0u;
+    __syncthreads();
+    a2 = fmax(fmax(red[0], red[1]), fmax(red[2], red[3]));
+  }
   const double L2E = 1.4426950408889634;
   const double y_lo = H.low - H.prior_mu, y_hi = H.high - H.prior_mu;
   const double sig = sqrt(0.5 * L2E / a2);
@@ -817,12 +871,31 @@
   acc[l][j] = a;
   if (census && j == 0 && nlive) atomicAdd(&live_n, nlive);
   TabAcc ce{-INFINITY, 0.0}, cg{-INFINITY, 0.0};
-  for (int k = tid; k < K; k += kTabThreads) {
-    const double x = cf[coef_off(k, 0)], y = cf[coef_off(k, 1)], z = cf[coef_off(k, 2)];
-    const double ak = -z, mu = y / (2.0 * ak), cc = x + ak * mu * mu;
-    const double d = fmax(0.0, fmax(pl - mu, mu - ph)), df = fmax(mu - pl, ph - mu);
-    tab_add(ce, cc + 8.0 * log2(2.0 * ak / L2E) - 0.5 * ak * d * d);
-    tab_add(cg, cc - ak * df * df);
+  if constexpr (LEAN) {
+    const TabTerm *__restrict__ tt = terms + (int64_t)slot * kcap;
+    for (int k = tid; k < K; k += 2 * kTabThreads) {
+      const int k1 = k + kTabThreads;
+      const TabTerm t0 = tt[k], t1 = tt[min(k1, K - 1)];
+      double te0, tg0, te1, tg1;
+      tab_cert_terms(t0, pl, ph, te0, tg0);
+      tab_cert_terms(t1, pl, ph, te1, tg1);
+      if (!(tab_add_noop(ce, te0) && tab_add_noop(cg, tg0))) {
+        tab_add(ce, te0);
+        tab_add(cg, tg0);
+      }
+      if (k1 < K && !(tab_add_noop(ce, te1) && tab_add_noop(cg, tg1))) {
+        tab_add(ce, te1);
+        tab_add(cg, tg1);
+      }
+    }
+  } else {
+    for (int k = tid; k < K; k += kTabThreads) {
+      const double x = cf[coef_off(k, 0)], y = cf[coef_off(k, 1)], z = cf[coef_off(k, 2)];
+      const double ak = -z, mu = y / (2.0 * ak), cc = x + ak * mu * mu;
+      const double d = fmax(0.0, fmax(pl - mu, mu - ph)), df = fmax(mu - pl, ph - mu);
+      tab_add(ce, cc + 8.0 * log2(2.0 * ak / L2E) - 0.5 * ak * d * d);
+      tab_add(cg, cc - ak * df * df);
+    }
   }
   ce = tab_wave_sum(ce);
   cg = tab_wave_sum(cg);
@@ -873,6 +946,29 @@
   ok = ok && le == le && le < INFINITY && lg > -INFINITY && lg < INFINITY &&
        fmax(le, lr) + 1.0 <= lg - 28.0;
   if (ok) atomicAdd(&hdr[slot].ncert, 1u);
+  if (cert_out) {
+    double *c = cert_out + ((int64_t)slot * kTabMaxPanels + p) * 3;
+    c[0] = le;
+    c[1] = lr;
+    c[2] = lg;
+  }
+}
+
+__global__ __launch_bounds__(kTabThreads) void k_table_build(
+    const tpe_hp *__restrict__ hps, const MixInfo *__restrict__ info,
+    const Coef *__restrict__ coef, int64_t kcap, TabHdr *__restrict__ hdr,
+    TabPanel *__restrict__ tab, unsigned long long *__restrict__ census,
+    double *__restrict__ cert_out) {
+  table_build_body<false>(hps, info, coef, kcap, hdr, tab, census, nullptr, nullptr, cert_out);
+}
+__global__ __launch_bounds__(kTabThreads) __attribute__((amdgpu_waves_per_eu(6)))
+void k_table_build_lean(
+    const tpe_hp *__restrict__ hps, const MixInfo *__restrict__ info,
+    const Coef *__restrict__ coef, int64_t kcap, TabHdr *__restrict__ hdr,
+    TabPanel *__restrict__ tab, unsigned long long *__restrict__ census,
+    const TabTerm *__restrict__ terms, const double *__restrict__ a2s,
+    double *__restrict__ cert_out) {
+  table_build_body<true>(hps, info, coef, kcap, hdr, tab, census, terms, a2s, cert_out);
 }
 
 constexpr int kBndThreads = 256;
@@ -960,14 +1056,25 @@
   bound[(int64_t)hp * kBndCells + cell] = ok ? U : INFINITY;
 }
 
+static_assert(sizeof(TabTerm) == kTabTermDoubles * sizeof(double), "terms scratch");
 hipError_t launch_table_build(const tpe_hp *hps, int32_t n_hp, const MixInfo *info,
                               const Coef *coef, int64_t kcap, TabHdr *hdr, TabPanel *tab,
-                              unsigned long long *census, hipStream_t st, double *bound) {
+                              unsigned long long *census, hipStream_t st, double *bound,
+                              double *terms, double *cert) {
   if (n_hp <= 0) return hipSuccess;
   hipError_t e = hipMemsetAsync(hdr, 0, (size_t)2 * n_hp * sizeof(TabHdr), st);
   if (e != hipSuccess) return e;
-  k_table_build<<<dim3(kTabMaxPanels, 2 * n_hp), kTabThreads, 0, st>>>(hps, info, coef, kcap, hdr,
-                                                                       tab, census);
+  const dim3 gb(kTabMaxPanels, 2 * n_hp);
+  if (terms) {
+    TabTerm *tt = reinterpret_cast<TabTerm *>(terms);
+    double *a2s = terms + (int64_t)2 * n_hp * kcap * kTabTermDoubles;
+    k_table_terms<<<dim3((unsigned)((kcap + kTabThreads - 1) / kTabThreads), 2 * n_hp), kTabThreads,
+                    0, st>>>(hps, info, coef, kcap, tt, a2s);
+    k_table_build_lean<<<gb, kTabThreads, 0, st>>>(hps, info, coef, kcap, hdr, tab, census, tt, a2s,
+                                                   cert);
+  } else {
+    k_table_build<<<gb, kTabThreads, 0, st>>>(hps, info, coef, kcap, hdr, tab, census, cert);
+  }
   if (bound)
     k_table_bound<<<dim3(kBndCells / kBndThreads, n_hp), kBndThreads, 0, st>>>(hps, hdr, tab, bound);
   return hipGetLastError();
diff --git a/hyperopt_amd/csrc/tpe_level_plan.hpp b/hyperopt_amd/csrc/tpe_level_plan.hpp
--- a/hyperopt_amd/csrc/tpe_level_plan.hpp
+++ b/hyperopt_amd/csrc/tpe_level_plan.hpp
@@ -153,11 +153,13 @@
   bool capturing = false;
   bool publish = false;
   int32_t screen_run = 0;
+  bool table_lean = true;
   bool operator==(const StepShape &o) const {
     return n_sug == o.n_sug && n_cand == o.n_cand && cand_begin == o.cand_begin &&
            n_total == o.n_total && below == o.below && fit == o.fit &&
            prune_mode == o.prune_mode && lattice_on == o.lattice_on &&
-           capturing == o.capturing && publish == o.publish && screen_run == o.screen_run;
+           capturing == o.capturing && publish == o.publish && screen_run == o.screen_run &&
+           table_lean == o.table_lean;
   }
 };
 inline int32_t step_screen_run(const Switches &sw) {
diff --git a/hyperopt_amd/csrc/tpe_score.hip b/hyperopt_amd/csrc/tpe_score.hip
--- a/hyperopt_amd/csrc/tpe_score.hip
+++ b/hyperopt_amd/csrc/tpe_score.hip
@@ -2376,6 +2376,89 @@
   }
 }
 
+template <bool CENSUS>
+__global__ __launch_bounds__(kWaves * 64) void k_table_map_dp_lean(ScoreArgs A) {
+  constexpr int KR = kMapRows, PW = kMapDpTiles / kWaves;
+  static_assert(PW == 64, "a wave's tile mask: one entry per lane");
+  __shared__ int wcnt[kWaves];
+  __shared__ int live[kMapDpTiles];
+  const int b = blockIdx.x;
+  int g = 0, b0 = 0;
+  for (; g + 1 < A.n_groups; ++g) {
+    const int nb = table_map_dp_blocks(A, g);
+    if (b < b0 + nb) break;
+    b0 += nb;
+  }
+  const int ntw = A.grp_tiles[g] * kWaves, nsb = (ntw + kMapDpTiles - 1) / kMapDpTiles;
+  const int local = b - b0;
+  int slot = A.grp_slot0[g] + local / nsb;
+  const int s = blockIdx.y;
+  if (A.compact) {
+    slot = active_slot(A, s, A.grp_slot0[g], A.grp_slots[g], local / nsb);
+    if (slot < 0) return;
+  }
+  const int hp = A.level_hps[slot];
+  const int64_t sb = 2 * (int64_t)hp, sa = sb + 1;
+  if (!(tab_valid(A.tab_hdr[sb]) && tab_valid(A.tab_hdr[sa]))) return;
+  if (!(A.force_active || A.compact ||
+        hp_active(A.hps[hp], A.results + (int64_t)s * A.n_hp, A.cond_parent, A.cond_branch)))
+    return;
+  const bool logn = A.grp_kind[g] == KIND_LSE_LW;
+  const double mu = A.hps[hp].prior_mu;
+  const int wave = __builtin_amdgcn_readfirstlane((int)(threadIdx.x >> 6));
+  const int lane = threadIdx.x & 63;
+  double *__restrict__ wmax = A.tab_wmax + ((int64_t)s * A.n_hp + hp) * A.pstride * kWaves;
+  const int wt0 = (local % nsb) * kMapDpTiles + wave;
+  const int wl = wt0 + kWaves * lane;
+  const bool in = wl < ntw;
+  const bool drop = in && (int64_t)wl * (64 * KR) < A.n_cand && wmax[wl] == -INFINITY;
+  const bool run = in && !drop;
+  const uint64_t todo = __ballot(run);
+  if constexpr (CENSUS) {
+    uint64_t dr = __ballot(drop);
+    while (dr) {
+      const int wt = wt0 + kWaves * (int)__builtin_ctzll(dr);
+      dr &= dr - 1;
+      if (lane == 0) {
+        const unsigned long long c =
+            (unsigned long long)min<int64_t>(64 * KR, A.n_cand - (int64_t)wt * (64 * KR)) *
+            (unsigned long long)(A.info[sb].K + A.info[sa].K);
+        atomicAdd(A.census + 3, c);
+        atomicAdd(A.census + 12, c);
+      }
+    }
+  }
+  if (lane == 0) wcnt[wave] = __popcll(todo);
+  __syncthreads();
+  int before = 0, total = 0;
+#pragma unroll
+  for (int w = 0; w < kWaves; ++w) {
+    const int c = wcnt[w];
+    before += w < wave ? c : 0;
+    total += c;
+  }
+  if (run) live[before + __popcll(todo & (((uint64_t)1 << lane) - 1))] = wl;
+  __syncthreads();
+  total = __builtin_amdgcn_readfirstlane(total);
+  if (wave >= total) return;
+  int wt = __builtin_amdgcn_readfirstlane(live[wave]);
+  double x[KR];
+  table_wave_load(A, s, slot, logn, wt, x);
+  for (int e = wave; e < total; e += kWaves) {
+    const bool more = e + kWaves < total;
+    const int wn = more ? __builtin_amdgcn_readfirstlane(live[e + kWaves]) : wt;
+    double xn[KR];
+    if (more) table_wave_load(A, s, slot, logn, wn, xn);
+    const double best = table_wave_tile<CENSUS, true>(A, s, hp, logn, wt, mu, x);
+    if (lane == 0) wmax[wt] = best;
+    if (more) {
+#pragma unroll
+      for (int r = 0; r < KR; ++r) x[r] = xn[r];
+    }
+    wt = wn;
+  }
+}
+
 constexpr int kPilotThreads = 1024;
 __global__ __launch_bounds__(kPilotThreads) void k_table_pilot(ScoreArgs A) {
   constexpr int NW = kPilotThreads / 64;
@@ -2562,6 +2645,138 @@
     if (base == 0 && !A.accumulate) A.results[sh] = Partial{NAN, NAN, -1, 1, 0};
   }
 }
+__global__ __launch_bounds__(kGatherThreads) void k_tie_gather_lean(ScoreArgs A) {
+  constexpr int NW = kGatherThreads / 64;
+  constexpr int WC = 64 * tile_rows(KIND_LSE_GW);
+  static_assert(tile_rows(KIND_LSE_GW) == tile_rows(KIND_LSE_LW), "one wave-tile shape");
+  __shared__ double red_s[NW];
+  __shared__ int red_n[NW];
+  __shared__ int wsum[NW];
+  const int s = blockIdx.y, tid = threadIdx.x, lane = tid & 63, wave = tid >> 6;
+  int row = blockIdx.x;
+  const int g = row_group(A, row);
+  const int nt = A.grp_tiles[g];
+  int slot = A.grp_slot0[g] + row;
+  if (A.compact) {
+    if (row == 0 && tid < 64) {
+      Partial *res = A.results + (int64_t)s * A.n_hp;
+      for (int i = tid; i < A.grp_slots[g]; i += 64) {
+        const int hp = A.level_hps[A.grp_slot0[g] + i];
+        if (!hp_active(A.hps[hp], res, A.cond_parent, A.cond_branch)) {
+          res[hp] = Partial{NAN, NAN, -1, 0, 0};
+          A.tie_cnt[(int64_t)s * A.n_hp + hp] = 0;
+        }
+      }
+    }
+    slot = active_slot(A, s, A.grp_slot0[g], A.grp_slots[g], row);
+    if (slot < 0) return;
+  }
+  const int hp = A.level_hps[slot];
+  const int64_t sh = (int64_t)s * A.n_hp + hp;
+  const bool act = A.force_active || A.compact ||
+                   hp_active(A.hps[hp], A.results + (int64_t)s * A.n_hp, A.cond_parent,
+                             A.cond_branch);
+  if (!act) {
+    if (tid == 0) {
+      A.results[sh] = Partial{NAN, NAN, -1, 0, 0};
+      A.tie_cnt[sh] = 0;
+    }
+    return;
+  }
+  const int ntw = nt * kWaves;
+  int32_t *list = A.tie_list + sh * A.pstride * kWaves;
+  if (!(tab_valid(A.tab_hdr[2 * (int64_t)hp]) && tab_valid(A.tab_hdr[2 * (int64_t)hp + 1]))) {
+    const int SBB = (1 << A.sort_log2) / tile_cands(KIND_LSE_GW);
+    for (int e = tid; e < ntw; e += kGatherThreads) {
+      const int j = e / kWaves, w = e % kWaves;
+      const int sb = j / SBB, q = j % SBB;
+      const int nbs = min(SBB, nt - sb * SBB);
+      list[e] = sb * SBB * kWaves + q + nbs * w;
+    }
+    if (tid == 0) A.tie_cnt[sh] = ntw;
+    return;
+  }
+  const double *wm = A.tab_wmax + sh * A.pstride * kWaves;
+  const int nrec = (int)min<int64_t>(ntw, (A.n_cand + WC - 1) / WC);
+  double m = -INFINITY;
+  int nan = 0;
+  constexpr int GB = 8;
+  const int nrow = (ntw + 63) / 64, rpw = (nrow + NW - 1) / NW;
+  const int r0 = min(wave * rpw, nrow), r1 = min(r0 + rpw, nrow);
+  auto load_rows = [&](int r, int lim, double fill, double (&v)[GB]) {
+#pragma unroll
+    for (int j = 0; j < GB; ++j) {
+      const int i = (r + j) * 64 + lane;
+      const double x = wm[min(i, lim - 1)];
+      v[j] = (r + j < r1 && i < lim) ? x : fill;
+    }
+  };
+  if (nrec > 0) {
+    for (int r = r0; r < r1; r += GB) {
+      double v[GB];
+      load_rows(r, nrec, -INFINITY, v);
+#pragma unroll
+      for (int j = 0; j < GB; ++j) {
+        nan |= v[j] != v[j];
+        m = fmax(m, v[j]);
+      }
+    }
+  }
+#pragma unroll
+  for (int o = 32; o > 0; o >>= 1) {
+    m = fmax(m, __shfl_xor(m, o, 64));
+    nan |= __shfl_xor(nan, o, 64);
+  }
+  if (lane == 0) { red_s[wave] = m; red_n[wave] = nan; }
+  __syncthreads();
+  m = red_s[0];
+  nan = red_n[0];
+#pragma unroll
+  for (int w = 1; w < NW; ++w) { m = fmax(m, red_s[w]); nan |= red_n[w]; }
+  const double tm = (nan || nrec <= 0) ? NAN : m;
+  if (tid == 0) A.tab_max[sh] = tm;
+  const double wthr = tm - A.tab_tie * fmax(1.0, fabs(tm));
+  const bool dp = A.tab_pref == 2;
+  int32_t *__restrict__ lw = list;
+  auto hot_of = [&](int i, double v) {
+    return i < ntw && !(v < wthr) && !(dp && i < nrec && v == -INFINITY);
+  };
+  int cnt = 0;
+  for (int r = r0; r < r1; r += GB) {
+    double v[GB];
+    load_rows(r, ntw, 0.0, v);
+#pragma unroll
+    for (int j = 0; j < GB; ++j)
+      cnt += __popcll(__ballot(r + j < r1 && hot_of((r + j) * 64 + lane, v[j])));
+  }
+  if (lane == 0) wsum[wave] = cnt;
+  __syncthreads();
+  int run = 0, total = 0;
+#pragma unroll
+  for (int w = 0; w < NW; ++w) {
+    const int c = wsum[w];
+    run += w < wave ? c : 0;
+    total += c;
+  }
+  if (cnt) {
+    for (int r = r0; r < r1; r += GB) {
+      double v[GB];
+      load_rows(r, ntw, 0.0, v);
+#pragma unroll
+      for (int j = 0; j < GB; ++j) {
+        const int i = (r + j) * 64 + lane;
+        const bool hot = r + j < r1 && hot_of(i, v[j]);
+        const uint64_t bal = __ballot(hot);
+        if (hot) lw[run + __popcll(bal & (((uint64_t)1 << lane) - 1))] = i;
+        run += __popcll(bal);
+      }
+    }
+  }
+  if (tid == 0) {
+    A.tie_cnt[sh] = total;
+    if (total == 0 && !A.accumulate) A.results[sh] = Partial{NAN, NAN, -1, 1, 0};
+  }
+}
 template <bool CENSUS, int MW>
 __global__ __launch_bounds__(kWaves * 64) __attribute__((amdgpu_waves_per_eu(TPE_WAVE_EU)))
 void k_score_wave1(ScoreArgs A) {
@@ -2790,6 +3005,7 @@
 constexpr int kTieBlocksPerCu = 16;
 
 static bool table_scalar_on() { return switches().table_scalar; }
+static bool table_lean_on() { return switches().table_lean; }
 
 static hipError_t launch_class(const ScoreArgs &a, int cls, bool has_erf, hipStream_t st) {
   if (a.n_groups <= 0) return hipSuccess;
@@ -2835,8 +3051,13 @@
         int32_t mb = 0;
         for (int i = 0; i < a.n_groups; ++i) mb += table_map_dp_blocks(a, i);
         const dim3 gm((unsigned)mb, a.n_suggest);
-        if (a.census) k_table_map_dp<true><<<gm, kWaves * 64, 0, st>>>(a);
-        else k_table_map_dp<false><<<gm, kWaves * 64, 0, st>>>(a);
+        if (table_lean_on()) {
+          if (a.census) k_table_map_dp_lean<true><<<gm, kWaves * 64, 0, st>>>(a);
+          else k_table_map_dp_lean<false><<<gm, kWaves * 64, 0, st>>>(a);
+        } else {
+          if (a.census) k_table_map_dp<true><<<gm, kWaves * 64, 0, st>>>(a);
+          else k_table_map_dp<false><<<gm, kWaves * 64, 0, st>>>(a);
+        }
       } else if (table_scalar_on()) {
         int32_t mb = 0;
         for (int i = 0; i < a.n_groups; ++i) mb += table_map_blocks(a, i);
@@ -2847,7 +3068,10 @@
         if (a.census) k_score_table<true, true><<<g, kWaves * 64, 0, st>>>(a);
         else k_score_table<false, true><<<g, kWaves * 64, 0, st>>>(a);
       }
-      k_tie_gather<<<dim3((unsigned)rows, a.n_suggest), kGatherThreads, 0, st>>>(a);
+      if (table_lean_on())
+        k_tie_gather_lean<<<dim3((unsigned)rows, a.n_suggest), kGatherThreads, 0, st>>>(a);
+      else
+        k_tie_gather<<<dim3((unsigned)rows, a.n_suggest), kGatherThreads, 0, st>>>(a);
       const int64_t per = ((int64_t)kTieBlocksPerCu * kNumCUs + (int64_t)rows * a.n_suggest - 1) /
                           ((int64_t)rows * a.n_suggest);
       const unsigned G = (unsigned)std::max<int64_t>(1, std::min<int64_t>(ntmax, per));
diff --git a/hyperopt_amd/csrc/tpe_switches.hpp b/hyperopt_amd/csrc/tpe_switches.hpp
--- a/hyperopt_amd/csrc/tpe_switches.hpp
+++ b/hyperopt_amd/csrc/tpe_switches.hpp
@@ -20,6 +20,7 @@
   bool draw_screen_int;
   bool table_prefilter;
   bool table_scalar;
+  bool table_lean;
   bool small_sort;
   bool side_streams;
   bool graph;
@@ -76,6 +77,7 @@
       {"TPE_DRAW_SCREEN_INT", R::OffIfNonEmptyZero, 1, &S::draw_screen_int, nullptr, 0, 0},
       {"TPE_TABLE_PREFILTER", R::OffIfNonEmptyZero, 1, &S::table_prefilter, nullptr, 0, 0},
       {"TPE_TABLE_SCALAR", R::OffIfNonEmptyZero, 1, &S::table_scalar, nullptr, 0, 0},
+      {"TPE_TABLE_LEAN", R::OffIfNonEmptyZero, 1, &S::table_lean, nullptr, 0, 0},
       {"TPE_SMALL_SORT", R::OnIfNonZero, 0, &S::small_sort, nullptr, 0, 0},
       {"TPE_SIDE_STREAMS", R::OnIfSet, 0, &S::side_streams, nullptr, 0, 0},
       {"TPE_GRAPH", R::OnIfSet, 0, &S::graph, nullptr, 0, 0},
diff --git a/hyperopt_amd/csrc/tpe_tab_add.hpp b/hyperopt_amd/csrc/tpe_tab_add.hpp
--- /dev/null
+++ b/hyperopt_amd/csrc/tpe_tab_add.hpp
@@ -0,0 +1,34 @@
+#pragma once
+#include <cmath>
+
+#if defined(__HIPCC__) || defined(__CUDACC__)
+#define TPE_TAB_HD __host__ __device__ inline __attribute__((always_inline))
+#else
+#define TPE_TAB_HD inline
+#endif
+
+namespace tpe {
+
+struct TabAcc {
+  double m, s;
+};
+
+TPE_TAB_HD void tab_add(TabAcc &a, double t) {
+  const double mn = fmax(a.m, ceil(t));
+  a.s = ldexp(a.s, (int)fmax(a.m - mn, -2100.0));
+  a.m = mn;
+  a.s += exp2(t - (mn == -INFINITY ? 0.0 : mn));
+}
+
+constexpr double kTabAddSkip = -56.0;
+
+TPE_TAB_HD bool tab_add_noop(const TabAcc &a, double t) {
+  return fabs(a.m) < INFINITY && t - a.m < kTabAddSkip;
+}
+
+TPE_TAB_HD void tab_add_skip(TabAcc &a, double t) {
+  if (tab_add_noop(a, t)) return;
+  tab_add(a, t);
+}
+
+}
diff --git a/include/tpe_engine.h b/include/tpe_engine.h
--- a/include/tpe_engine.h
+++ b/include/tpe_engine.h
@@ -228,6 +228,10 @@
 int tpe_plan_tie_counts(tpe_plan_t p, int32_t n_suggest, int32_t *counts);
 int tpe_plan_tab_wmax(tpe_plan_t p, int32_t n_suggest, double *out);
 int tpe_plan_tab_bound(tpe_plan_t p, int32_t hp, double *out);
+int tpe_plan_tab_panels(tpe_plan_t p, int32_t hp, int32_t side, double *y_lo, double *inv_w,
+                        int32_t *ncert, void *panels);
+int tpe_plan_tab_cert(tpe_plan_t p, int32_t hp, int32_t side, double *out);
+int tpe_plan_tie_list(tpe_plan_t p, int32_t s, int32_t hp, int32_t *out);
 int tpe_plan_tab_hot(tpe_plan_t p, int32_t n_suggest, double *out);
 int64_t tpe_plan_cand_dump(tpe_plan_t p, int32_t s, int32_t hp, double *values,
                            int32_t *positions);
```

Measured after the change: 1274000 billion pairs/s (median of 6 runs). 5.3% higher.
